# SunYangtian/UniGeo

Measured on AMD Instinct MI355X. Metric: frames/sec (384x512, 25-frame clip, 25 denoise steps), higher is better.
Workload: dtype fp16; 1 GPU; DepthCrafter SVD-UNet fp16, 25-step Euler, 25-frame 384x512 clips (BASELINE configs[1]); CLIP + VAE enc/dec + depth post-proc inside the timed region; one clip per ug_dc_run call, one call at a time (SURVEY 8d; reference eval.py:33-39); frames=25, height=384, width=512, denoise_steps=25, parallelism=clip-sharded x1, RCCL all_gather of depth, clips_in_flight_per_gpu=1, lanes=1

## Files before the change

unigeo_amd/_lib.py:

```python
import ctypes as C
import dataclasses
import json
import os

import numpy as np

_HERE = os.path.dirname(os.path.abspath(__file__))
LIB_PATH = os.environ.get("UG_LIB_PATH") or os.path.join(_HERE, "csrc", "libunigeo_hip.so")

EXPORTS = [
    "ug_unet_config_default", "ug_vae_config_default", "ug_clip_config_default",
    "ug_create", "ug_destroy", "ug_last_error", "ug_workspace_peak",
    "ug_load_tensor", "ug_bind_unet", "ug_bind_vae", "ug_bind_clip",
    "ug_dc_set_inputs", "ug_dc_run", "ug_dc_run_windows", "ug_dc_get_outputs", "ug_dc_device_ptrs", "ug_dc_set_trace", "ug_dc_set_guidance", "ug_unet_forward_pair", "ug_dc_set_inputs_ex", "ug_dc_get_noise", "ug_op_philox_u32", "ug_op_randn", "ug_op_u8_to_frames", "ug_set_vae_encode_fp32", "ug_set_concurrency", "ug_set_coscheduled", "ug_set_fp8_linears", "ug_op_linear_mx8", "ug_set_ff_fused", "ug_op_ff", "ug_op_ln_ff", "ug_bench_ff", "ug_bench_flash", "ug_tune_flash", "ug_tune_ff",
    "ug_eval_depth", "ug_eval_normal", "ug_depth_eval_opts_default", "ug_eval_depth_ex", "ug_eval_depth_global", "ug_op_masked_median", "ug_clip_embed", "ug_vae_encode", "ug_vae_decode", "ug_unet_forward", "ug_normals_from_depth",
    "ug_op_linear", "ug_op_conv", "ug_op_conv_gn", "ug_op_groupnorm", "ug_op_layernorm", "ug_op_flash_attn",
    "ug_op_temporal_attn", "ug_op_attention_generic", "ug_op_flash_attn_dh", "ug_op_euler_step", "ug_op_flash_cross_attn", "ug_op_temporal_attn_nv",
    "ug_op_split_pair", "ug_op_gn32_pair", "ug_op_conv_wide", "ug_op_attn_wide",
    "ug_bind_stablenormal", "ug_sn_run", "ug_sn_unet_forward", "ug_sn_dino", "ug_sn_vae_decode", "ug_sn_vae_encode", "ug_resize_bilinear",
    "ug_pcd_opts_default", "ug_pcd_world_points", "ug_eval_pcd", "ug_op_pcd_nn", "ug_op_pcd_select", "ug_op_pcd_knn_normals", "ug_eval_pcd_fps", "ug_op_pcd_fps",
    "ug_eval_pcd_ex", "ug_op_pcd_nn_grid", "ug_op_pcd_knn_normals_grid",
    "ug_pointmap_opts_default", "ug_pointmap_focal", "ug_pointmap_poses",
    "ug_vis_depth_range", "ug_vis_panels", "ug_prep_resize_frames", "ug_prep_gt", "ug_prep_gt_ex",
    "ug_profile_begin", "ug_profile_begin_shapes", "ug_profile_end", "ug_bench_gemm", "ug_bench_groupnorm", "ug_bench_mfma_peak", "ug_tune_force",
]


class UNetConfigC(C.Structure):
    _fields_ = [("in_channels", C.c_int), ("out_channels", C.c_int), ("num_levels", C.c_int),
                ("block_out_channels", C.c_int * 8), ("num_attention_heads", C.c_int * 8),
                ("down_has_attn", C.c_int * 8),
                ("layers_per_block", C.c_int), ("cross_attention_dim", C.c_int),
                ("addition_time_embed_dim", C.c_int), ("projection_class_embeddings_input_dim", C.c_int),
                ("norm_groups", C.c_int),
                ("eps_cross_attn_blocks", C.c_float), ("eps_plain_down_block", C.c_float),
                ("eps_mid_block", C.c_float), ("eps_up_blocks", C.c_float)]


class VAEConfigC(C.Structure):
    _fields_ = [("in_channels", C.c_int), ("out_channels", C.c_int), ("latent_channels", C.c_int),
                ("num_levels", C.c_int), ("block_out_channels", C.c_int * 8),
                ("layers_per_block", C.c_int), ("norm_groups", C.c_int), ("scaling_factor", C.c_float)]


class CLIPConfigC(C.Structure):
    _fields_ = [("hidden_size", C.c_int), ("intermediate_size", C.c_int), ("num_hidden_layers", C.c_int),
                ("num_attention_heads", C.c_int), ("image_size", C.c_int), ("patch_size", C.c_int),
                ("projection_dim", C.c_int), ("layer_norm_eps", C.c_float)]


class DepthEvalOptsC(C.Structure):
    _fields_ = [("alignment", C.c_int), ("max_depth", C.c_float), ("pre_clip_min", C.c_float), ("pre_clip_max", C.c_float),
                ("post_clip_min", C.c_float), ("post_clip_max", C.c_float)]


class PcdOptsC(C.Structure):
    _fields_ = [("threshold", C.c_float), ("max_iteration", C.c_int), ("knn", C.c_int)]


class PointmapOptsC(C.Structure):
    _fields_ = [("reproj_px", C.c_double), ("max_iter", C.c_int), ("max_rounds", C.c_int)]


DEPTH_ALIGNMENTS = {"lstsq": 0, "median": 1, "scale": 2, "metric": 3}
PREP_DEPTH_F64, PREP_ZOOMED = 1, 2

_lib = None


def _set_argtypes(lib, table):
    try:
        for name, argtypes in table.items():
            getattr(lib, name).argtypes = argtypes
    except AttributeError:
        if not os.environ.get("UG_LIB_PATH"):
            raise


def load_library():
    global _lib
    if _lib is not None:
        return _lib
    if not os.path.exists(LIB_PATH):
        raise RuntimeError(
            f"{LIB_PATH} not found: build it with `python -c 'import __graft_entry__ as g; g.build()'` "
            "(or `make -C unigeo_amd/csrc`).  The MI355X path has no CPU / PyTorch fallback.")
    lib = C.CDLL(LIB_PATH)
    fp, ip, vp = C.POINTER(C.c_float), C.c_int, C.c_void_p
    lib.ug_create.restype = vp
    lib.ug_create.argtypes = [ip, C.c_size_t, C.c_size_t]
    lib.ug_destroy.argtypes = [vp]
    lib.ug_last_error.restype = C.c_char_p
    lib.ug_last_error.argtypes = [vp]
    lib.ug_workspace_peak.restype = C.c_size_t
    lib.ug_workspace_peak.argtypes = [vp]
    lib.ug_load_tensor.argtypes = [vp, C.c_char_p, ip, ip, C.POINTER(C.c_int64), vp]
    lib.ug_bind_unet.argtypes = [vp, C.POINTER(UNetConfigC)]
    lib.ug_bind_vae.argtypes = [vp, C.POINTER(VAEConfigC)]
    lib.ug_bind_clip.argtypes = [vp, C.POINTER(CLIPConfigC)]
    lib.ug_dc_set_inputs.argtypes = [vp, vp, ip, ip, ip, vp, vp, vp]
    lib.ug_dc_run.argtypes = [vp, ip, ip, ip]
    lib.ug_dc_run_windows.argtypes = [vp, ip, ip, ip, ip, ip]
    lib.ug_dc_get_outputs.argtypes = [vp, vp, vp, vp]
    lib.ug_dc_set_trace.argtypes = [vp, vp, ip]
    lib.ug_set_vae_encode_fp32.argtypes = [vp, ip]
    _set_argtypes(lib, {
        "ug_set_fp8_linears": [vp, ip], "ug_set_concurrency": [vp, ip], "ug_set_coscheduled": [vp, ip], "ug_set_ff_fused": [vp, ip],
        "ug_bench_ff": [vp, ip, ip, ip, ip, vp], "ug_bench_flash": [vp, ip, ip, ip, ip, ip, vp], "ug_tune_flash": [vp, ip], "ug_tune_ff": [vp, ip],
        "ug_op_ff": [vp, vp, ip, ip, vp, vp, vp, vp, vp, C.c_float, C.c_float, ip, vp],
        "ug_op_ln_ff": [vp, vp, ip, ip, vp, vp, C.c_float, vp, ip, vp, vp, vp, vp, C.c_float, C.c_float, ip, vp],
        "ug_op_linear_mx8": [vp, vp, ip, ip, vp, ip, vp, ip, vp, vp, vp]})
    _set_argtypes(lib, {"ug_dc_set_guidance": [vp, C.c_float], "ug_unet_forward_pair": [vp, vp, vp, vp, vp, ip, ip, ip, C.c_float, vp, vp]})
    _set_argtypes(lib, {
        "ug_dc_set_inputs_ex": [vp, vp, ip, ip, ip, ip, vp, vp, C.c_uint64, vp], "ug_dc_get_noise": [vp, vp, vp],
        "ug_op_philox_u32": [vp, C.c_uint64, C.c_uint32, C.c_uint64, C.c_long, vp],
        "ug_op_randn": [vp, C.c_uint64, C.c_uint32, C.c_uint64, C.c_long, C.c_long, vp], "ug_op_u8_to_frames": [vp, vp, ip, ip, ip, vp]})
    lib.ug_dc_device_ptrs.argtypes = [vp, C.POINTER(vp), C.POINTER(vp), C.POINTER(vp)]
    lib.ug_eval_depth.argtypes = [vp, vp, vp, vp, C.c_long, C.c_float, vp]
    lib.ug_eval_normal.argtypes = [vp, vp, vp, vp, C.c_long, vp]
    lib.ug_depth_eval_opts_default.restype = None
    lib.ug_depth_eval_opts_default.argtypes = [C.POINTER(DepthEvalOptsC)]
    lib.ug_eval_depth_ex.argtypes = [vp, vp, vp, vp, C.c_long, C.POINTER(DepthEvalOptsC), vp, vp]
    lib.ug_eval_depth_global.argtypes = [vp, vp, vp, vp, vp, vp, vp, ip, ip, ip, C.POINTER(DepthEvalOptsC), vp, vp]
    lib.ug_op_masked_median.argtypes = [vp, vp, vp, C.c_long, C.c_float, C.c_float, C.c_float, vp, C.POINTER(C.c_long)]
    lib.ug_pcd_opts_default.restype = None
    _set_argtypes(lib, {"ug_pcd_opts_default": [C.POINTER(PcdOptsC)],
                        "ug_pcd_world_points": [vp, vp, vp, vp, vp, ip, ip, ip, C.POINTER(DepthEvalOptsC), vp, vp],
                        "ug_eval_pcd": [vp, vp, vp, vp, C.c_long, vp, C.c_long, C.POINTER(PcdOptsC), vp, vp, vp],
                        "ug_op_pcd_nn": [vp, vp, C.c_long, vp, C.c_long, vp, vp, vp],
                        "ug_op_pcd_select": [vp, vp, ip, C.c_long, C.c_long, vp],
                        "ug_op_pcd_knn_normals": [vp, vp, C.c_long, ip, vp, vp]})
    _set_argtypes(lib, {"ug_eval_pcd_fps": [vp, vp, vp, vp, C.c_long, C.c_long, C.POINTER(PcdOptsC), vp, vp, vp, vp, vp],
                        "ug_op_pcd_fps": [vp, vp, C.c_long, C.c_long, vp, vp]})
    _set_argtypes(lib, {"ug_eval_pcd_ex": [vp, vp, vp, vp, C.c_long, vp, C.c_long, C.POINTER(PcdOptsC), ip, vp, vp, vp, vp, vp, vp],
                        "ug_op_pcd_nn_grid": [vp, vp, C.c_long, vp, C.c_long, vp, vp, vp, vp],
                        "ug_op_pcd_knn_normals_grid": [vp, vp, C.c_long, ip, vp, vp, vp]})
    _set_argtypes(lib, {"ug_pointmap_opts_default": [C.POINTER(PointmapOptsC)],
                        "ug_pointmap_focal": [vp, vp, ip, ip, C.c_double, C.c_double, vp],
                        "ug_pointmap_poses": [vp, vp, vp, ip, ip, ip, C.c_double, C.c_double, C.c_double, C.POINTER(PointmapOptsC), vp, vp, vp, vp]})
    if hasattr(lib, "ug_pointmap_opts_default"):
        lib.ug_pointmap_opts_default.restype = None
    _set_argtypes(lib, {"ug_vis_depth_range": [vp, vp, C.c_long, vp],
                        "ug_vis_panels": [vp, vp, vp, vp, ip, ip, ip, ip, C.c_float, C.c_float, vp, vp, ip, vp]})
    _set_argtypes(lib, {"ug_prep_resize_frames": [vp, vp, ip, ip, ip, ip, ip, vp, vp, ip, vp, vp, ip, vp],
                        "ug_prep_gt": [vp, vp, C.c_float, vp, vp, vp, ip, ip, ip, vp, ip, vp, ip, C.c_float, vp, vp, vp, vp, vp],
                        "ug_prep_gt_ex": [vp, vp, C.c_float, vp, vp, vp, ip, ip, ip, vp, ip, vp, ip, C.c_float, vp, vp, vp, vp, vp, C.c_uint]})
    lib.ug_clip_embed.argtypes = [vp, vp, ip, ip, ip, vp]
    lib.ug_vae_encode.argtypes = [vp, vp, ip, ip, ip, vp]
    lib.ug_vae_decode.argtypes = [vp, vp, ip, ip, ip, vp]
    lib.ug_unet_forward.argtypes = [vp, vp, ip, ip, ip, C.c_float, vp, vp]
    lib.ug_normals_from_depth.argtypes = [vp, vp, vp, ip, ip, ip, vp]
    lib.ug_op_linear.argtypes = [vp, vp, ip, ip, vp, ip, vp, vp, C.c_float, C.c_float, ip, ip, vp]
    lib.ug_op_conv.argtypes = [vp, vp, ip, vp, ip, ip, ip, ip, vp, vp, ip, ip, ip, ip, ip, ip, ip, vp]
    lib.ug_op_groupnorm.argtypes = [vp, vp, ip, vp, ip, ip, ip, ip, C.c_float, ip, ip, vp, vp, vp]
    lib.ug_op_conv_gn.argtypes = [vp, vp, ip, ip, ip, ip, vp, vp, vp, ip, ip, ip, ip, C.c_float, ip, vp, vp, vp, vp, vp, vp]
    lib.ug_op_layernorm.argtypes = [vp, vp, ip, ip, C.c_float, vp, vp, vp, ip, vp, vp]
    lib.ug_op_flash_attn.argtypes = [vp, vp, ip, ip, ip, vp]
    lib.ug_op_temporal_attn.argtypes = [vp, vp, ip, ip, ip, vp]
    lib.ug_op_attention_generic.argtypes = [vp, vp, ip, ip, ip, ip, vp]
    lib.ug_op_flash_attn_dh.argtypes = [vp, vp, ip, ip, ip, ip, vp]
    lib.ug_op_euler_step.argtypes = [vp, vp, vp, C.c_long, C.c_float, C.c_float]
    _set_argtypes(lib, {"ug_op_flash_cross_attn": [vp, vp, vp, ip, ip, ip, ip, ip, C.c_long, C.c_long, C.c_long, C.c_long, vp],
                        "ug_op_temporal_attn_nv": [vp, vp, ip, ip, ip, ip, vp]})
    _set_argtypes(lib, {
        "ug_op_split_pair": [vp, vp, C.c_long, ip, vp, vp], "ug_op_gn32_pair": [vp, vp, ip, ip, ip, ip, C.c_float, ip, vp, vp, vp, vp],
        "ug_op_conv_wide": [vp, vp, ip, ip, ip, ip, vp, vp, ip, vp, ip, ip, ip, ip, ip, vp], "ug_op_attn_wide": [vp, vp, ip, ip, ip, vp]})
    lib.ug_bind_stablenormal.argtypes = [vp, C.POINTER(UNetConfigC), C.POINTER(VAEConfigC), C.POINTER(CLIPConfigC)]
    lib.ug_sn_run.argtypes = [vp, vp, ip, ip, ip, vp, C.c_float, ip, vp, vp, vp, vp]
    lib.ug_sn_unet_forward.argtypes = [vp, ip, vp, vp, ip, ip, ip, C.c_float, C.c_float, vp, vp, ip, vp]
    lib.ug_sn_dino.argtypes = [vp, vp, ip, ip, ip, vp]
    lib.ug_sn_vae_decode.argtypes = [vp, vp, ip, ip, ip, vp]
    lib.ug_sn_vae_encode.argtypes = [vp, vp, ip, ip, ip, vp]
    lib.ug_resize_bilinear.argtypes = [vp, vp, ip, ip, ip, ip, ip, ip, ip, vp]
    lib.ug_profile_begin.argtypes = [vp]
    lib.ug_bench_gemm.argtypes = [vp] + [ip] * 16 + [vp]
    lib.ug_bench_groupnorm.argtypes = [vp, ip, ip, ip, ip, ip, ip, ip, vp]
    lib.ug_bench_mfma_peak.argtypes = [vp, ip, vp]
    lib.ug_tune_force.argtypes = [vp, ip, ip]
    lib.ug_profile_begin_shapes.argtypes = [vp]
    lib.ug_profile_end.restype = C.c_char_p
    lib.ug_profile_end.argtypes = [vp]
    _lib = lib
    return lib


def _f32(a):
    return np.ascontiguousarray(a, dtype=np.float32)


def _ptr(a):
    return None if a is None else a.ctypes.data_as(C.c_void_p)


def _fill8(dst, vals):
    for i in range(8):
        dst[i] = int(vals[i]) if i < len(vals) else 0


def _unet_c(cfg):
    c = UNetConfigC()
    c.in_channels, c.out_channels, c.num_levels = cfg.in_channels, cfg.out_channels, len(cfg.block_out_channels)
    _fill8(c.block_out_channels, cfg.block_out_channels)
    _fill8(c.num_attention_heads, cfg.num_attention_heads)
    _fill8(c.down_has_attn, [int(b) for b in cfg.down_has_attn])
    c.layers_per_block, c.cross_attention_dim, c.norm_groups = cfg.layers_per_block, cfg.cross_attention_dim, cfg.norm_groups
    for name in ("addition_time_embed_dim", "projection_class_embeddings_input_dim",
                 "eps_cross_attn_blocks", "eps_plain_down_block", "eps_mid_block", "eps_up_blocks"):
        setattr(c, name, getattr(cfg, name, 0))
    return c


def _vae_c(cfg):
    c = VAEConfigC()
    c.in_channels, c.out_channels, c.latent_channels = cfg.in_channels, cfg.out_channels, cfg.latent_channels
    c.num_levels = len(cfg.block_out_channels)
    _fill8(c.block_out_channels, cfg.block_out_channels)
    c.layers_per_block, c.norm_groups, c.scaling_factor = cfg.layers_per_block, cfg.norm_groups, cfg.scaling_factor
    return c


def _clip_c(cfg):
    c = CLIPConfigC()
    c.hidden_size, c.intermediate_size = cfg.hidden_size, cfg.intermediate_size
    c.num_hidden_layers, c.num_attention_heads = cfg.num_hidden_layers, cfg.num_attention_heads
    c.image_size, c.patch_size, c.layer_norm_eps = cfg.image_size, cfg.patch_size, cfg.layer_norm_eps
    c.projection_dim = getattr(cfg, "projection_dim", 0)
    return c


class Engine:

    def __init__(self, device_id=0, workspace_bytes=2 << 30, persist_bytes=1 << 30):
        self.lib = load_library()
        self.ctx = self.lib.ug_create(int(device_id), int(workspace_bytes), int(persist_bytes))
        if not self.ctx:
            raise RuntimeError("ug_create failed: " + self.lib.ug_last_error(None).decode())
        self.device_id = device_id

    def close(self):
        if getattr(self, "ctx", None):
            self.lib.ug_destroy(self.ctx)
            self.ctx = None

    def __del__(self):
        try:
            self.close()
        except Exception:
            pass

    def _ck(self, rc):
        if rc != 0:
            raise RuntimeError("libunigeo_hip: " + self.lib.ug_last_error(self.ctx).decode())

    def load_state(self, prefix, state):
        for name, arr in state.items():
            a = np.ascontiguousarray(arr)
            if a.dtype == np.float16:
                dt = 0
            elif a.dtype == np.float32:
                dt = 1
            else:
                a = a.astype(np.float32); dt = 1
            shape = (C.c_int64 * max(a.ndim, 1))(*(a.shape if a.ndim else (1,)))
            self._ck(self.lib.ug_load_tensor(self.ctx, (prefix + name).encode(), dt, max(a.ndim, 1), shape, _ptr(a)))

    def bind_unet(self, cfg):
        self._ck(self.lib.ug_bind_unet(self.ctx, C.byref(_unet_c(cfg))))
        self.unet_cfg = cfg

    def bind_vae(self, cfg):
        self._ck(self.lib.ug_bind_vae(self.ctx, C.byref(_vae_c(cfg))))
        self.vae_cfg = cfg

    def bind_clip(self, cfg):
        self._ck(self.lib.ug_bind_clip(self.ctx, C.byref(_clip_c(cfg))))
        self.clip_cfg = cfg

    def bind_stablenormal(self, ucfg, vcfg, dcfg):
        self._ck(self.lib.ug_bind_stablenormal(self.ctx, C.byref(_unet_c(ucfg)), C.byref(_vae_c(vcfg)), C.byref(_clip_c(dcfg))))
        self.sn_cfgs = (ucfg, vcfg, dcfg)

    def sn_run(self, images, prompt_embeds, yoso_t, timesteps, ca, cb):
        f = _f32(images); B, H, W, _ = f.shape
        pe = _f32(prompt_embeds).reshape(77, self.sn_cfgs[0].cross_attention_dim)
        ts, a, b = _f32(timesteps), _f32(ca), _f32(cb)
        out = np.empty((B, H, W, 3), np.float32)
        self._ck(self.lib.ug_sn_run(self.ctx, _ptr(f), B, H, W, _ptr(pe), float(yoso_t), int(ts.size), _ptr(ts), _ptr(a), _ptr(b), _ptr(out)))
        return out

    def sn_unet_forward(self, which, sample, t_unet, prompt_embeds, zimg=None, t_ctrl=0.0, dino_tokens=None, use_ctrl=False):
        s = _f32(sample); B, _, h, w = s.shape
        z = None if zimg is None else _f32(zimg)
        d = None if dino_tokens is None else _f32(dino_tokens)
        pe = _f32(prompt_embeds)
        out = np.empty((B, 4, h, w), np.float32)
        self._ck(self.lib.ug_sn_unet_forward(self.ctx, int(which), _ptr(s), _ptr(z), B, h, w, float(t_unet), float(t_ctrl), _ptr(pe), _ptr(d),
                                             int(bool(use_ctrl)), _ptr(out)))
        return out

    def sn_dino(self, images):
        f = _f32(images); B, H, W, _ = f.shape
        dc = self.sn_cfgs[2]; g = dc.image_size // dc.patch_size
        out = np.empty((B, g * g, dc.hidden_size), np.float32)
        self._ck(self.lib.ug_sn_dino(self.ctx, _ptr(f), B, H, W, _ptr(out)))
        return out

    def sn_vae_decode(self, z):
        z = _f32(z); B, _, h, w = z.shape
# ... 402 lines not shown
        return out[0]

    def op_pcd_knn_normals(self, pts, knn=30):
        p = np.ascontiguousarray(np.asarray(pts, np.float64).reshape(-1, 3))
        nbr, nrm = np.empty((len(p), min(knn, len(p))), np.int32), np.empty((len(p), 3), np.float64)
        self._ck(self.lib.ug_op_pcd_knn_normals(self.ctx, _ptr(p), len(p), int(knn), _ptr(nbr), _ptr(nrm)))
        return nbr, nrm

    def op_masked_median(self, pred, gt, max_depth=80.0, pre_clip_min=None, pre_clip_max=None):
        p, g = _f32(pred).reshape(-1), _f32(gt).reshape(-1)
        med = np.zeros(2, np.float32); cnt = C.c_long(0)
        nan = float("nan")
        self._ck(self.lib.ug_op_masked_median(self.ctx, _ptr(p), _ptr(g), p.size, nan if max_depth is None else float(max_depth),
                                              nan if pre_clip_min is None else float(pre_clip_min),
                                              nan if pre_clip_max is None else float(pre_clip_max), _ptr(med), C.byref(cnt)))
        return med[0], med[1], int(cnt.value)

    def eval_normal(self, gt, mask=None, pred=None):
        g = _f32(gt); n = g.size // 3
        p = None if pred is None else _f32(pred)
        m = None if mask is None else np.ascontiguousarray(np.asarray(mask).astype(np.uint8))
        out = np.zeros(8, np.float64)
        self._ck(self.lib.ug_eval_normal(self.ctx, _ptr(p), _ptr(g), _ptr(m), n, _ptr(out)))
        return dict(zip(self.NORMAL_KEYS, out.tolist()))

    VIS_RGB_NONE, VIS_RGB_HOST, VIS_RGB_RESIDENT = 0, 1, 2

    def vis_depth_range(self, depth=None):
        out = np.zeros(2, np.float32)
        if depth is None:
            T, H, W = self._shape
            self._ck(self.lib.ug_vis_depth_range(self.ctx, None, T * H * W, _ptr(out)))
        else:
            d = _f32(depth)
            self._ck(self.lib.ug_vis_depth_range(self.ctx, _ptr(d), d.size, _ptr(out)))
        return out[0], out[1]

    def vis_panels(self, vmin, vmax, lut, depth=None, normals=None, rgbs=None, cbar=None):
        d = None if depth is None else _f32(depth)
        n = None if normals is None else _f32(normals)
        if d is not None:
            shape = d.shape
        elif n is not None:
            shape = n.shape[:3]
        else:
            shape = self._shape
        if len(shape) != 3 or (n is not None and n.shape != (*shape, 3)):
            raise ValueError("vis_panels: depth must be [T,H,W] and normals [T,H,W,3]")
        T, H, W = shape
        r, mode = None, self.VIS_RGB_NONE
        if isinstance(rgbs, str):
            if rgbs != "resident":
                raise ValueError('vis_panels: rgbs must be None, "resident" or an array')
            mode = self.VIS_RGB_RESIDENT
        elif rgbs is not None:
            r, mode = _f32(rgbs), self.VIS_RGB_HOST
            if r.shape != (T, H, W, 3):
                raise ValueError("vis_panels: rgbs must be [T,H,W,3]")
        l = _f32(lut)
        if l.shape != (256, 3):
            raise ValueError("vis_panels: lut must be [256,3]")
        cb, Wc = None, 0
        if cbar is not None:
            cb = _f32(cbar)
            if cb.ndim != 3 or cb.shape[0] != H or cb.shape[2] != 3:
                raise ValueError("vis_panels: cbar must be [H,Wc,3]")
            Wc = cb.shape[1]
        Wp = (W if mode else 0) + 2 * W + (5 + Wc if cb is not None else 0)
        out = np.empty((T, H, Wp, 3), np.uint8)
        self._ck(self.lib.ug_vis_panels(self.ctx, _ptr(d), _ptr(n), _ptr(r), mode, T, H, W, float(vmin), float(vmax), _ptr(l), _ptr(cb), Wc, _ptr(out)))
        return out

    def prep_resize_frames(self, frames_u8, Ho, Wo, row_taps=None, col_taps=None):
        from .harness.scannetpp import resize_taps
        f = np.asarray(frames_u8)
        if f.dtype != np.uint8 or f.ndim != 4 or f.shape[3] != 3:
            raise ValueError("prep_resize_frames: frames must be uint8 [T,Hi,Wi,3]")
        f = np.ascontiguousarray(f)
        T, Hi, Wi, _ = f.shape
        Ho, Wo = int(Ho), int(Wo)
        tabs = []
        for taps, n_in, n_out in ((row_taps, Hi, Ho), (col_taps, Wi, Wo)):
            idx, w = resize_taps(n_in, n_out) if taps is None else taps
            idx, w = np.ascontiguousarray(idx, dtype=np.int32), np.ascontiguousarray(w, dtype=np.float64)
            if idx.ndim != 2 or idx.shape != w.shape or idx.shape[0] != n_out:
                raise ValueError("prep_resize_frames: a tap table must be (idx, w), both [n_out, K]")
            tabs.append((idx, w))
        (ri, rw), (ci, cw) = tabs
        out = np.empty((T, 3, Ho, Wo), np.float32)
        self._ck(self.lib.ug_prep_resize_frames(self.ctx, _ptr(f), T, Hi, Wi, Ho, Wo, _ptr(ri), _ptr(rw), ri.shape[1], _ptr(ci), _ptr(cw),
                                                ci.shape[1], _ptr(out)))
        return out

    def prep_gt(self, depth_u16, normals_u8, intrinsics, cam2key, row_idx, col_idx, depth_divisor=1000.0, max_depth=80.0, depth_f64=False,
                zoomed=None):
        d = np.asarray(depth_u16)
        if d.dtype != np.uint16 or d.ndim != 3:
            raise ValueError("prep_gt: depth must be uint16 [T,Hi,Wi]")
        d = np.ascontiguousarray(d)
        T, Hi, Wi = d.shape
        n = None
        if normals_u8 is not None:
            n = np.asarray(normals_u8)
            if n.dtype != np.uint8 or n.shape != (T, Hi, Wi, 3):
                raise ValueError("prep_gt: normals must be uint8 [T,Hi,Wi,3]")
            n = np.ascontiguousarray(n)
        k, m = _f32(intrinsics).reshape(T, 3, 3), _f32(cam2key).reshape(T, 4, 4)
        ri, ci = np.ascontiguousarray(row_idx, dtype=np.int32).reshape(-1), np.ascontiguousarray(col_idx, dtype=np.int32).reshape(-1)
        Ho, Wo = ri.size, ci.size
        cn, cc, wn, wc = (np.empty((T, 3, Ho, Wo), np.float32) for _ in range(4))
        mask = np.empty((T, Ho, Wo), np.float32)
        if zoomed is None:
            zoomed = (Ho, Wo) != (Hi, Wi)
        flags = (PREP_DEPTH_F64 if depth_f64 else 0) | (PREP_ZOOMED if zoomed else 0)
        self._ck(self.lib.ug_prep_gt_ex(self.ctx, _ptr(d), float(depth_divisor), _ptr(n), _ptr(k), _ptr(m), T, Hi, Wi, _ptr(ri), Ho, _ptr(ci), Wo,
                                        float(max_depth), _ptr(cn), _ptr(cc), _ptr(wn), _ptr(wc), _ptr(mask), flags))
        return cn, cc, wn, wc, mask

    def op_linear(self, A, W, bias=None, R1=None, c0=1.0, c1=1.0, act=0, geglu=False):
        A, W = _f32(A), _f32(W); M, K = A.shape; N = W.shape[0]
        b = None if bias is None else _f32(bias); r = None if R1 is None else _f32(R1)
        out = np.empty((M, N // 2 if geglu else N), np.float32)
        self._ck(self.lib.ug_op_linear(self.ctx, _ptr(A), M, K, _ptr(W), N, _ptr(b), _ptr(r), c0, c1, act, int(geglu), _ptr(out)))
        return out

    def op_conv(self, x0, weight, bias=None, x1=None, kt=1, k=3, stride=1, pad_t=1, pad_l=1, ups=1):
        x0 = _f32(x0); T, H, W, C0 = x0.shape
        x1a = None if x1 is None else _f32(x1); C1 = 0 if x1 is None else x1a.shape[-1]
        w = _f32(weight); O = w.shape[0]
        b = None if bias is None else _f32(bias)
        Ho, Wo = H * ups // stride, W * ups // stride
        out = np.empty((T, Ho, Wo, O), np.float32)
        self._ck(self.lib.ug_op_conv(self.ctx, _ptr(x0), C0, _ptr(x1a), C1, T, H, W, _ptr(w), _ptr(b), O, kt, k,
                                     stride, pad_t, pad_l, ups, _ptr(out)))
        return out

    def op_groupnorm(self, x0, G, eps, gamma, beta, x1=None, temporal=False, silu=False):
        x0 = _f32(x0); T, HW, C0 = x0.shape
        x1a = None if x1 is None else _f32(x1); C1 = 0 if x1 is None else x1a.shape[-1]
        out = np.empty((T, HW, C0 + C1), np.float32)
        self._ck(self.lib.ug_op_groupnorm(self.ctx, _ptr(x0), C0, _ptr(x1a), C1, T, HW, G, eps, int(temporal), int(silu),
                                          _ptr(_f32(gamma)), _ptr(_f32(beta)), _ptr(out)))
        return out

    def op_conv_gn(self, x, w, b, G, eps, gamma, beta, res=None, kt=1, k=3, temporal=False):
        x = _f32(x); T, H, W, C0 = x.shape; w = _f32(w); O = w.shape[0]
        r = None if res is None else _f32(res)
        co = np.empty((T, H, W, O), np.float32); y1 = np.empty_like(co); y2 = np.empty_like(co)
        rb = C.c_int(0)
        self._ck(self.lib.ug_op_conv_gn(self.ctx, _ptr(x), C0, T, H, W, _ptr(w), _ptr(None if b is None else _f32(b)), _ptr(r), O, kt, k, G, eps, int(temporal),
                                        _ptr(_f32(gamma)), _ptr(_f32(beta)), _ptr(co), _ptr(y1), _ptr(y2), C.byref(rb)))
        return co, y1, y2, rb.value

    def op_layernorm(self, x, eps, gamma, beta, addvec=None, rows_per_vec=1):
        x = _f32(x); M, Cc = x.shape
        out = np.empty((M, Cc), np.float32); xout = np.empty((M, Cc), np.float32)
        av = None if addvec is None else _f32(addvec)
        self._ck(self.lib.ug_op_layernorm(self.ctx, _ptr(x), M, Cc, eps, _ptr(_f32(gamma)), _ptr(_f32(beta)), _ptr(av),
                                          rows_per_vec, _ptr(out), _ptr(xout)))
        return (out, xout) if addvec is not None else out

    def op_flash_attn(self, qkv, B, H, S):
        q = _f32(qkv); out = np.empty((B * S, H * 64), np.float32)
        self._ck(self.lib.ug_op_flash_attn(self.ctx, _ptr(q), B, H, S, _ptr(out)))
        return out

    def op_temporal_attn(self, qkv, T, HW, H):
        q = _f32(qkv); out = np.empty((T * HW, H * 64), np.float32)
        self._ck(self.lib.ug_op_temporal_attn(self.ctx, _ptr(q), T, HW, H, _ptr(out)))
        return out

    def op_flash_cross_attn(self, q, kv, out_inout, B, H, S, Sk=0, kv_shared=False, guard=0):
        q, kv, out = _f32(q), _f32(kv), np.array(out_inout, dtype=np.float32, order="C")
        keys = Sk if Sk > 0 else S
        assert q.ndim == kv.ndim == out.ndim == 2 and q.shape[0] == B * S and out.shape[0] == B * S + guard, (q.shape, kv.shape, out.shape)
        assert Sk < 0 or kv.shape[0] == (1 if kv_shared else B) * keys + guard, kv.shape
        self._ck(self.lib.ug_op_flash_cross_attn(self.ctx, _ptr(q), _ptr(kv), B, H, S, Sk, int(bool(kv_shared)), q.shape[1], kv.shape[1], out.shape[1],
                                                 int(guard), _ptr(out)))
        return out

    def op_temporal_attn_nv(self, qkv, nv, T, HW, H):
        q = _f32(qkv); out = np.empty((nv * T * HW, H * 64), np.float32)
        assert q.shape == (nv * T * HW, 3 * H * 64), q.shape
        self._ck(self.lib.ug_op_temporal_attn_nv(self.ctx, _ptr(q), nv, T, HW, H, _ptr(out)))
        return out

    def op_attention_generic(self, qkv, B, S, H, d):
        q = _f32(qkv); out = np.empty((B * S, H * d), np.float32)
        self._ck(self.lib.ug_op_attention_generic(self.ctx, _ptr(q), B, S, H, d, _ptr(out)))
        return out

    def op_flash_attn_dh(self, qkv, B, S, H, d):
        q = _f32(qkv); out = np.empty((B * S, H * d), np.float32)
        self._ck(self.lib.ug_op_flash_attn_dh(self.ctx, _ptr(q), B, S, H, d, _ptr(out)))
        return out

    def op_split_pair(self, x):
        x = _f32(x); M, Cc = x.shape
        hi = np.empty((M, Cc), np.float32); lo = np.empty((M, Cc), np.float32)
        self._ck(self.lib.ug_op_split_pair(self.ctx, _ptr(x), M, Cc, _ptr(hi), _ptr(lo)))
        return hi, lo

    def op_gn32_pair(self, x, G, eps, gamma, beta, silu=False):
        x = _f32(x); T, HW, Cc = x.shape
        hi = np.empty((T, HW, Cc), np.float32); lo = np.empty((T, HW, Cc), np.float32)
        self._ck(self.lib.ug_op_gn32_pair(self.ctx, _ptr(x), T, HW, Cc, G, eps, int(silu), _ptr(_f32(gamma)), _ptr(_f32(beta)), _ptr(hi), _ptr(lo)))
        return hi, lo

    def op_conv_wide(self, x, weight, bias=None, res=None, res_in_place=False, k=3, stride=1, pad_t=1, pad_l=1):
        x = _f32(x); T, H, W, Cc = x.shape
        w = _f32(weight); O = w.shape[0]
        b = None if bias is None else _f32(bias); r = None if res is None else _f32(res)
        out = np.empty((T, H // stride, W // stride, O), np.float32)
        self._ck(self.lib.ug_op_conv_wide(self.ctx, _ptr(x), T, H, W, Cc, _ptr(w), _ptr(b), O, _ptr(r), int(bool(res_in_place)), k, stride, pad_t, pad_l, _ptr(out)))
        return out

    def op_attn_wide(self, qkv, T, S):
        q = _f32(qkv); Cc = q.shape[1] // 3
        out = np.empty((T * S, Cc), np.float32)
        self._ck(self.lib.ug_op_attn_wide(self.ctx, _ptr(q), T, S, Cc, _ptr(out)))
        return out

    def op_euler_step(self, v, lat, sigma, sigma_next):
        v = _f32(v); l = _f32(lat).copy()
        self._ck(self.lib.ug_op_euler_step(self.ctx, _ptr(v), _ptr(l), l.size, sigma, sigma_next))
        return l

    def bench_gemm(self, M=0, N=0, K=0, conv=None, cfg=-1, split=0, iters=20):
        out = np.zeros(8, np.float32)
        cv = conv or {}
        self._ck(self.lib.ug_bench_gemm(self.ctx, M, N, K, int(conv is not None), cv.get("T", 0), cv.get("H", 0), cv.get("W", 0),
                                        cv.get("C0", 0), cv.get("C1", 0), cv.get("kt", 1), cv.get("k", 1), cv.get("stride", 1),
                                        cv.get("ups", 1), cfg, split, iters, _ptr(out)))
        Mr, Kr = float(out[3]), float(out[4])
        return float(out[0]), 2.0 * Mr * N * Kr / (out[0] * 1e-3) / 1e12, int(out[1]), int(out[2])

    def bench_mfma_peak(self, iters=20000):
        out = np.zeros(1, np.float32)
        self._ck(self.lib.ug_bench_mfma_peak(self.ctx, int(iters), _ptr(out)))
        return float(out[0])

    def tune_force(self, cfg=-1, split=-1):
        self._ck(self.lib.ug_tune_force(self.ctx, int(cfg), int(split)))

    def bench_groupnorm(self, C0, C1, T, HW, temporal, mode, iters=20):
        out = np.zeros(1, np.float32)
        self._ck(self.lib.ug_bench_groupnorm(self.ctx, C0, C1, T, HW, int(temporal), mode, iters, _ptr(out)))
        return float(out[0])

    def profile_begin(self, shapes=False):
        self._ck((self.lib.ug_profile_begin_shapes if shapes else self.lib.ug_profile_begin)(self.ctx))

    def profile_end(self):
        prof = json.loads(self.lib.ug_profile_end(self.ctx).decode())
        self.last_profile_order = prof.pop("__order__", None)
        return prof

    def workspace_peak(self):
        return int(self.lib.ug_workspace_peak(self.ctx))
```

unigeo_amd/csrc/common.h:

```cpp
#pragma once
#include <hip/hip_runtime.h>
#include <hip/hip_fp16.h>
#include <stdint.h>
#include <stdio.h>
#include <stdexcept>
#include <string>

typedef _Float16 f16;
typedef _Float16 f16x2 __attribute__((ext_vector_type(2)));
typedef _Float16 f16x4 __attribute__((ext_vector_type(4)));
typedef _Float16 f16x8 __attribute__((ext_vector_type(8)));
typedef float f32x4 __attribute__((ext_vector_type(4)));
typedef float f32x16 __attribute__((ext_vector_type(16)));

#define UG_CHECK(expr)                                                                        \
  do {                                                                                        \
    hipError_t _e = (expr);                                                                   \
    if (_e != hipSuccess)                                                                     \
      throw std::runtime_error(std::string(#expr) + " failed: " + hipGetErrorString(_e) +    \
                               " at " + __FILE__ + ":" + std::to_string(__LINE__));           \
  } while (0)

#define UG_REQUIRE(cond, msg)                                                                 \
  do {                                                                                        \
    if (!(cond))                                                                              \
      throw std::runtime_error(std::string("requirement failed: ") + #cond + " : " + (msg) + \
                               " at " + __FILE__ + ":" + std::to_string(__LINE__));           \
  } while (0)

static inline int cdiv(long a, long b) { return (int)((a + b - 1) / b); }
static inline int ug_dev_slot() { int d = 0; (void)hipGetDevice(&d); return d & 31; }

enum { UG_ACT_NONE = 0, UG_ACT_SILU = 1, UG_ACT_GELU = 2 };
enum { UG_F_GEGLU = 1, UG_F_OUT_F32 = 2, UG_F_NOXCD = 4, UG_F_PRIO = 8 ,
       UG_F_XCDROUND = 32 ,
       UG_F_R1_F32 = 16  };

struct GemmP {
  const f16* A0; const f16* A1;
  int C0, C1;
  int M, N, K;
  int conv;
  int T, Hi, Wi, Ho, Wo;
  int ups, stride, pad_t, pad_l;
  int kt, ky, kx;
  const f16* W; long ldw;
  const f16* bias; const f16* bias2;
  const f16* R1; long ldr1; float c1;
  const f16* R2; long ldr2; float c2;
  float c0;
  void* Out; long ldo;
  int act, flags;
  const f16* zero;
  int nb_inner;
  long sA_o, sA_i, sW_o, sW_i, sO_o, sO_i;
  int cfg_p1;
  int splitk;
  float* partial;
  void* trace;
  int up_phase;
  const unsigned* sa; const unsigned* sw; long ld_sa, ld_sw;
  int kchunk;
  int tm_T, tm_nb;
  int m_off;
  int group_m;
  int halo_tw, halo_lg;
  int tune_cfg_p1, tune_split_p1, tune_knobs;
  float2* stat_part; int stat_hw;
};
struct GemmTune { int cfg = -1, split = -1, knobs = 0; };
static inline void gemm_apply_tune(GemmP& p, const GemmTune& t) { p.tune_cfg_p1 = t.cfg + 1; p.tune_split_p1 = t.split + 1; p.tune_knobs = t.knobs; }
void launch_gemm_mx8(const GemmP& p, hipStream_t s);
void launch_quant_mx8(const f16* x, long ldx, long M, int K, unsigned char* q, unsigned* scales, long ld_s, hipStream_t s);
void launch_gemm(const GemmP& p, int batch, hipStream_t s, int* stat_rb = nullptr);
bool gemm_stream_supported(const GemmP& p, int batch);
void launch_gemm_stream(const GemmP& p, hipStream_t s);
bool conv_halo_supported(const GemmP& p, int batch, int bm, int bn);
void launch_conv_halo(const GemmP& p, int bm, int bn, hipStream_t s);
void gemm_plan(const GemmP& p, int batch, int* cfg_out, int* split_out);

struct FFusedP {
  const f16* X; const f16* W1; const f16* b1; const f16* W2; const f16* b2;
  const f16* R1; const f16* R2; float c0, c1, c2;
  f16* Out; int M, C; const f16* zero;
  const f16* ln_g; const f16* ln_b; float ln_eps; const f16* addvec; int rows_per_vec;
  int variant;
};
bool ff_fused_supported(int C);
void launch_ff_fused(const FFusedP& p, hipStream_t s);

struct GroupNormP {
  const f16* X0; const f16* X1; int C0, C1;
  int T, HW, G; float eps; int temporal; int silu;
  const f16* gamma; const f16* beta;
  f16* Y;
  float* ws;
  int mode;
  const float2* part; int part_rb;
};
bool launch_groupnorm(const GroupNormP& p, hipStream_t s);
bool groupnorm_uses_part(const GroupNormP& p, int part_rb);
size_t groupnorm_ws_floats(int T, int HW, int C, int G);

struct LayerNormP {
  const f16* X; f16* Y; int M, C; float eps;
  const f16* gamma; const f16* beta;
  const f16* addvec; int rows_per_vec; f16* Xout;
  long row0;
  unsigned char* Y8; unsigned* S8; long ld_s8;
};
void launch_layernorm(const LayerNormP& p, hipStream_t s);

struct FlashP {
  const f16* Q; const f16* K; const f16* V; long ldq, ldk, ldv;
  f16* O; long ldo;
  int B, H, S; float scale;
  int Sk = 0; int kv_shared = 0;
  int variant = -1;
};
void launch_flash_attn64(const FlashP& p, hipStream_t s);
bool flash_attn_dh_supported(int d);
void launch_flash_attn_dh(const FlashP& p, int d, hipStream_t s);

struct TemporalAttnP {
  const f16* Q; const f16* K; const f16* V; long ld;
  f16* O; long ldo;
  int T, HW, H; float scale;
  int nv = 1;
};
void launch_temporal_attn64(const TemporalAttnP& p, hipStream_t s);

void launch_softmax_rows(const float* in, long ld_in, f16* out, long ld_out, long rows, int S,
                         hipStream_t s);
void launch_transpose(const f16* in, long ldi, long sbi, f16* out, long ldo, long sbo, int B, int R,
                      int C, int nb_inner, long sbi_inner, long sbo_inner, hipStream_t s);

void launch_cast_f32_f16(const float* in, f16* out, long n, hipStream_t s);
void launch_cast_f16_f32(const f16* in, float* out, long n, hipStream_t s);
void launch_permute_conv_w(const f16* in, f16* out, int O, int I, int taps, int Ipad, int Opad,
                           hipStream_t s);
void launch_upsample_phase_w(const f16* w9, f16* w4, int O, int I, int Ipad, hipStream_t s);
void launch_rechunk_conv_w(const f16* in, f16* out, long O, int taps, int Ipad, hipStream_t s);
void launch_gather_rows(const f16* in, f16* out, const int* rowmap, int rows, int cols, hipStream_t s);
void launch_copy2d(const f16* in, long ldi, f16* out, long ldo, long rows, int cols, hipStream_t s);
void launch_fill_f16(f16* p, float v, long n, hipStream_t s);
void launch_fill_random(f16* p, long n, unsigned seed, hipStream_t s);
void launch_add_rowvec(const f16* x, const f16* vec, f16* y, long M, int C, int rows_per_vec,
                       hipStream_t s);
void launch_axpby(const f16* a, const f16* b, f16* y, float ca, float cb, long n, hipStream_t s);

void launch_prep_video(const float* frames, const float* noise, f16* clip_src, f16* vae_in,
                       int T, int H, int W, float noise_aug, hipStream_t s);
void launch_clip_patchify(const f16* video_m11, f16* patches, int T, int H, int W, int S224,
                          int P, int Kpad, hipStream_t s, int imagenet_norm = 0);
void launch_scale_rows(f16* w, const f16* gamma, int N, int K, hipStream_t s);
void launch_add_grid_nearest(f16* x, const f16* grid, int B, int h, int w, int g, int C, hipStream_t s);
void launch_sn_normals_out(const f16* dec, int ldd, float* out, long pixels, hipStream_t s);
void launch_resize_bilinear_aa(const float* in, float* out, int B, int Hi, int Wi, int Ho, int Wo, int C, int normalise, hipStream_t s);
void launch_init_latents2(const float* noise, f16* lat, float sigma0, int T, long hw, hipStream_t s);
void launch_silu_f16(const f16* in, f16* out, long n, hipStream_t s);
void launch_clip_assemble(const f16* patches, const f16* cls, const f16* pos, f16* tok, int T, int np, int d,
                          hipStream_t s);
void launch_make_unet_input(const f16* lat, const f16* cond, f16* x, long pixels, float inv_scale,
                            hipStream_t s);
void launch_euler_step(const f16* v, f16* lat, long n, float sigma, float sigma_next, hipStream_t s);
void launch_make_unet_input_cfg(const f16* lat, const f16* cond, f16* x, long pixels, float inv_scale, hipStream_t s);
void launch_euler_step_cfg(const f16* vc, const f16* vu, float g, f16* lat, long n, float sigma, float sigma_next, hipStream_t s);
void launch_scale_f16(const f16* in, f16* out, float sc, long n, hipStream_t s);
void launch_axpby_f16(const f16* x, float a, const f16* y, float b, f16* out, long n, hipStream_t s);
void launch_crossfade_f16(const f16* cur, f16* all, long frame_elems, int overlap, hipStream_t s);
void launch_pad_channels(const f16* in, int Cin, f16* out, int Cout, long pixels, hipStream_t s);
void launch_time_conv_out(const f16* x, const f16* w, const f16* b, float* frames_out, int T,
                          long HW, int Cs, hipStream_t s);
void launch_depth_post(const float* frames, float* depth, float* minmax_ws, long pixels,
                       hipStream_t s);
void launch_normals(const float* depth, const float* K33, float* normals, int T, int H, int W,
                    hipStream_t s);

void launch_philox_u32(uint32_t* out, long nblocks, uint64_t seed, uint32_t stream, uint64_t q0, hipStream_t s);
void launch_randn(float* out, long n, uint64_t seed, uint32_t stream, uint64_t e0, hipStream_t s);
void launch_u8_to_frames(const unsigned char* in_tchw, float* out_thwc, int T, long HW, hipStream_t s);

void launch_split_pair(const float* x, f16* y, long M, int C, hipStream_t s);
void launch_add_f32(const float* a, const float* b, float* y, long n, hipStream_t s);
void launch_take_cols_f16(const float* x, long ldx, f16* y, long M, int C, hipStream_t s);
size_t gn32_ws_bytes(int T, int HW, int C, int G);
void launch_gn32_pair(const float* X, f16* Y, int T, int HW, int C, int G, float eps, int silu, const f16* gamma, const f16* beta,
                      void* ws, hipStream_t s);
void launch_qk_terms(const float* qkv, f16* Aq, f16* Bk, long M, int C, hipStream_t s);
void launch_vt_terms(const float* qkv, f16* Vt, int B, int S, int Spad, int C, hipStream_t s);
void launch_softmax_pair(const float* in, long ld_in, f16* out, int Spad, long rows, int S, float pscale, hipStream_t s);

float bench_mfma_peak(float* scratch, int iters, hipStream_t s);

void launch_depth_fit(const float* pred, const float* gt, long n, float max_depth, double* part, int* nb, hipStream_t s);
void launch_depth_metrics(const float* pred, const float* gt, const unsigned char* cmask, long n, float max_depth, float sc,
                          float sh, double* part, int* nb, hipStream_t s);
void launch_normal_err(const float* pn, const float* gn, const unsigned char* mask, long n, float* err, double* part,
                       unsigned* hist, int* nb, hipStream_t s);
void launch_collect_bin(const float* err, long n, int bin, float* out, unsigned* count, unsigned cap, hipStream_t s);
#define SEL_PREFIX 2048
#define SEL_RANK 2050
#define SEL_COUNT 2052
#define SEL_MED 2053
#define SEL_WORDS 2056
void launch_masked_median(const float* pred, const float* gt, long n, float max_depth, float lo, float hi, unsigned* sel, hipStream_t s);
void launch_weiszfeld_scale(const float* pred, const float* gt, long n, float max_depth, float lo, float hi, int iters, double* wz,
                            double* part, hipStream_t s);
void launch_depth_fit_ex(const float* pred, const float* gt, long n, float max_depth, float lo, float hi, double* part, int* nb, hipStream_t s);
void launch_depth_metrics_ex(const float* pred, const float* gt, const unsigned char* cmask, long n, float max_depth, float lo, float hi,
                             float plo, float phi, float sc, float sh, double* part, float* emap, int* nb, hipStream_t s);
void launch_world_radius(const float* pred, const float* gt, const float* gt_radius, const double* cam, long n, int H, int W, float max_depth,
                         float plo, float phi, float sc, float sh, float* radius, double* part, int* nb, hipStream_t s);
void launch_world_points(const float* pred, const double* cam, long n, int H, int W, float plo, float phi, float sc, float sh, float* pts,
                         hipStream_t s);
void launch_radius_metrics(const float* radius, const float* gt, const float* gt_radius, const unsigned char* cmask, long n, float max_depth,
                           float sc, float sh, double* part, float* rmap, int* nb, hipStream_t s);
#define PCD_MAXB 1024
#define PCD_SEL_WORDS 264
__host__ __device__ inline unsigned long long pcd_key(double f) {
  const unsigned long long u = __builtin_bit_cast(unsigned long long, f);
  return u ^ ((u >> 63) ? ~0ull : (1ull << 63));
}
__host__ __device__ inline unsigned long long pcd_key(float f) {
  const unsigned u = __builtin_bit_cast(unsigned, f);
  return (unsigned long long)(u ^ ((u >> 31) ? 0xffffffffu : 0x80000000u)) << 32;
}
__host__ __device__ inline double pcd_unkey_f64(unsigned long long k) {
  return __builtin_bit_cast(double, k ^ ((k >> 63) ? (1ull << 63) : ~0ull));
}
__host__ __device__ inline float pcd_unkey_f32(unsigned long long k) {
// ... 65 lines not shown
```

unigeo_amd/csrc/engine.h:

```cpp
#pragma once
#include <map>
#include <memory>
#include <string>
#include <unordered_map>
#include <vector>

#include "common.h"

namespace ug {

struct RawTensor { void* dev = nullptr; int dtype = 0; std::vector<long> shape; long numel = 0; bool used = false; };

class Arena {
 public:
  void init(size_t bytes);
  void destroy();
  void* alloc(size_t bytes);
  template <class T> T* get(long n) { return (T*)alloc((size_t)n * sizeof(T)); }
  size_t mark() const { return off_; }
  void release(size_t m) { off_ = m; }
  size_t peak() const { return peak_; }
  size_t capacity() const { return cap_; }
  void view(void* base, size_t bytes) { base_ = (char*)base; cap_ = bytes; off_ = 0; peak_ = 0; hi_ = 0; }
  void reset_high() { hi_ = off_; }
  size_t high() const { return hi_; }
  void note_peak(size_t p) { if (p > peak_) peak_ = p; }
 private:
  char* base_ = nullptr; size_t cap_ = 0, off_ = 0, peak_ = 0, hi_ = 0;
};

struct Lin { const f16* w = nullptr; const f16* b = nullptr; int in = 0, out = 0;
             const unsigned char* w8 = nullptr; const unsigned* sw8 = nullptr; long ld_sw8 = 0; };
struct Conv { const f16* w = nullptr; const f16* b = nullptr; int cin = 0, cinp = 0, cout = 0, kt = 1, ky = 1, kx = 1;
              const f16* wphase = nullptr;
              int kchunk = 0; };
struct Norm { const f16* g = nullptr; const f16* b = nullptr; int c = 0; float eps = 1e-5f; };

struct Res2D { Norm n1, n2; Conv c1, c2, sc; Lin temb; bool has_sc = false, has_temb = false; int tidx = -1; };
struct ResT { Norm n1, n2; Conv c1, c2; Lin temb; bool has_temb = false; int tidx = -1; };
struct STRes { Res2D s; ResT t; float alpha = 0.5f; int cin = 0, cout = 0; };

struct Transformer {
  int C = 0, heads = 0;
  Norm gn; Lin proj_in, proj_out;
  Norm ln1, ln3; Lin qkv1, o1, v2, o2, ff1, ff2;
  Norm ln_in, tln1, tln3; Lin ffin1, ffin2, tqkv, to1, tv2, to2, tff1, tff2;
  Lin tpe1, tpe2;
  float alpha = 0.5f;
  f16* frame_emb = nullptr; int frame_emb_T = 0;
  f16* cross_sp = nullptr;
  f16* cross_tm = nullptr;
};

struct UNetCfg {
  int in_ch = 8, out_ch = 4, nlev = 4; int boc[8] = {320, 640, 1280, 1280}; int heads[8] = {5, 10, 20, 20};
  int has_attn[8] = {1, 1, 1, 0}; int layers = 2, cross_dim = 1024, add_dim = 256, proj_in_dim = 768, groups = 32;
  float eps_xattn = 1e-6f, eps_down = 1e-5f, eps_mid = 1e-5f, eps_up = 1e-6f;
};
struct VAECfg { int in_ch = 3, out_ch = 3, lat = 4, nlev = 4; int boc[8] = {128, 256, 512, 512}; int layers = 2, groups = 32; float scaling = 0.18215f; };
struct CLIPCfg { int hidden = 1280, inter = 5120, layers = 32, heads = 16, image = 224, patch = 14, proj = 1024; float eps = 1e-5f; };

struct UNet {
  UNetCfg cfg; bool bound = false;
  Conv conv_in, conv_out; Norm norm_out;
  Lin te1, te2, ae1, ae2;
  struct Down { std::vector<STRes> res; std::vector<Transformer> attn; Conv down; bool has_down = false; };
  struct Up { std::vector<STRes> res; std::vector<Transformer> attn; Conv up; bool has_up = false; };
  std::vector<Down> down; std::vector<Up> up;
  STRes mid0, mid1; Transformer mid_attn;
  std::vector<Res2D*> temb_s; std::vector<ResT*> temb_t;
  f16* tproj = nullptr; long tproj_stride = 0; int tproj_steps = 0; std::vector<long> tproj_off_s, tproj_off_t;
  int prep_nv = 1;
};

struct VAttn { Norm gn; Lin qkv, out; int C = 0; };
struct VAE {
  VAECfg cfg; bool bound = false;
  Conv e_in, e_out, quant; Norm e_norm;
  struct EDown { std::vector<Res2D> res; Conv down; bool has_down = false; };
  std::vector<EDown> edown; Res2D emid0, emid1; VAttn eattn;
  std::vector<EDown> edown_w; Res2D emid0_w, emid1_w; VAttn eattn_w; Conv e_out_w, quant_w; bool wide_bound = false;
  Conv d_in, d_out; Norm d_norm; const f16* tco_w = nullptr; const f16* tco_b = nullptr;
  std::vector<STRes> dmid; VAttn dattn;
  struct DUp { std::vector<STRes> res; Conv up; bool has_up = false; };
  std::vector<DUp> dup;
  bool dec2d = false; Conv post_quant; std::vector<Res2D> d2_mid; std::vector<std::vector<Res2D>> d2_up;
};

struct CLIPLayer { Norm ln1, ln2; Lin qkv, out, fc1, fc2; };
struct CLIP {
  CLIPCfg cfg; bool bound = false;
  const f16* patch_w = nullptr; int patch_k = 0;
  const f16* patch_b = nullptr;
  const f16* cls = nullptr; const f16* pos = nullptr;
  Norm pre, post; std::vector<CLIPLayer> layers; Lin proj;
};

struct SDTransformer {
  int C = 0, heads = 0;
  Norm gn; Lin proj_in, proj_out; Norm ln1, ln2, ln3; Lin qkv1, o1, q2, kv2, o2, ff1, ff2;
  f16* kv = nullptr;
};
struct TembSet { std::vector<Res2D*> res; f16* tproj = nullptr; std::vector<long> off; int steps = 0; };
struct SDTrunk {
  Conv conv_in; Lin te1, te2;
  struct Down { std::vector<Res2D> res; std::vector<SDTransformer> attn; Conv down; bool has_down = false; };
  std::vector<Down> down; Res2D mid0, mid1; SDTransformer mid_attn;
};
struct SDUNetM {
  SDTrunk tr; TembSet ts;
  struct Up { std::vector<Res2D> res; std::vector<SDTransformer> attn; Conv up; bool has_up = false; };
  std::vector<Up> up; Norm norm_out; Conv conv_out;
};
struct ControlNetM { SDTrunk tr; TembSet ts; std::vector<Conv> zero; Conv zero_mid; Lin dino_proj; bool has_dino = false; };
struct SN {
  UNetCfg cfg; bool bound = false;
  SDUNetM unet_y, unet_r; ControlNetM ctrl_y, ctrl_d; VAE vae; CLIP dino;
};

struct ProfRec { std::string name; double flops, bytes; hipEvent_t e0, e1; };

struct Lane { hipStream_t stream = nullptr; hipEvent_t done = nullptr; };

struct Ctx {
  int device = 0; hipStream_t stream = nullptr;
  Arena ws;
  Arena persist;
  f16* zero = nullptr;
  std::string err;
  std::unordered_map<std::string, RawTensor> raw;
  UNet unet; VAE vae; CLIP clip; SN sn;
  bool prof_on = false; bool prof_shapes = false; std::vector<ProfRec> prof; std::string prof_json;
  int T = 0, H = 0, W = 0;
  float* d_frames = nullptr; float* d_noise_lat = nullptr; float* d_noise_aug = nullptr; float* d_K = nullptr;
  float* d_out_frames = nullptr; float* d_depth = nullptr; float* d_normals = nullptr; float* d_mm = nullptr;
  f16* d_clip_emb = nullptr; f16* d_cond = nullptr; f16* d_lat = nullptr;
  size_t io_mark = 0; bool io_ready = false;
  bool normals_ready = false;
  float* d_pcd_pts = nullptr; long pcd_cap = 0, pcd_pixels = 0;
  float* trace_host = nullptr; int trace_steps = 0;
  void* pin[2] = {nullptr, nullptr}; size_t pin_sz[2] = {0, 0};
  int ff_fused = 3;
  int fp8_linears = 0;
  int vae_encode_fp32 = 1;
  float guidance = 1.f;
  std::vector<Lane> lanes; hipEvent_t fork_ev = nullptr;
  int concurrency = 1;
  std::map<std::string, size_t> lane_need;
  int cur_lane = 0;
  int cosched = 0;
  int ff_variant = 0, flash_variant = -1;
  GemmTune tune;
};

void* pinned(Ctx& c, int slot, size_t bytes);

void upload_raw(Ctx& c, const std::string& name, int dtype, const std::vector<long>& shape, const void* host);
void bind_unet(Ctx& c, const UNetCfg& cfg, const std::string& prefix);
void bind_vae(Ctx& c, const VAECfg& cfg, const std::string& prefix);
void bind_clip(Ctx& c, const CLIPCfg& cfg, const std::string& prefix);
void finish_binding(Ctx& c, const std::string& prefix);
inline int geglu_src_row(int v, int inner) { const int blk = v / 16, wv = v % 16; return wv < 8 ? blk * 8 + wv : inner + blk * 8 + (wv - 8); }

void unet_prepare(Ctx& c, int T, const f16* clip_emb, const float* timesteps, int nsteps, int nv = 1);
f16* unet_forward(Ctx& c, const f16* x, int T, int h, int w, int step, int nv = 1, int vid0 = 0);
f16* vae_encode(Ctx& c, const f16* x8, int T, int H, int W);
void vae_decode(Ctx& c, const f16* z, int T, int h, int w, float* frames_out);
f16* clip_embed(Ctx& c, const f16* video_m11, int T, int H, int W);

f16* vae_encode_v(Ctx& c, VAE& v, const f16* x8, int T, int H, int W, bool fp32_grade);
void test_unfused_attention(Ctx& c, const f16* qkv, long ld, int B, int S, int H, int d, f16* out, long ldo);
void attn_wide_core(Ctx& c, const float* qkv, int T, int S, int C, float* ao);
void test_conv_wide(Ctx& c, const std::string& name, bool bias, const float* x, int T, int H, int W, int cin, int cout, int k, int stride, int pad_t, int pad_l,
                    float* out, const float* res);

void bind_sn(Ctx& c, const UNetCfg& ucfg, const VAECfg& vcfg, const CLIPCfg& dcfg, const std::string& prefix);
void sn_run(Ctx& c, const float* images, int B, int H, int W, const float* prompt, float yoso_t, int nsteps, const float* timesteps,
            const float* ca, const float* cb, float* normals_out);
f16* sn_unet_eval(Ctx& c, int which, const f16* sample4, const f16* zimg4, int B, int h, int w, float t_unet, float t_ctrl, const f16* prompt,
                  const f16* dino_tok, int use_ctrl);
f16* sn_dino_tokens(Ctx& c, const f16* img_m11, int B, int H, int W);
f16* sn_vae_decode(Ctx& c, const f16* z4, int B, int h, int w);

void dc_set_inputs(Ctx& c, const float* frames, int T, int H, int W, const float* noise_lat, const float* noise_aug,
                   const float* K33);
void dc_set_inputs_ex(Ctx& c, const void* frames, int frames_u8, int T, int H, int W, const float* noise_lat, const float* noise_aug,
                      uint64_t noise_seed, const float* K33);
void dc_get_noise(Ctx& c, float* noise_lat, float* noise_aug);
// ... 8 lines not shown
```

unigeo_amd/csrc/engine.hip:

```cpp
#include "engine.h"
#include <chrono>

#include <math.h>
#include <stdlib.h>
#include <string.h>

#include <algorithm>
#include <exception>
#include <sstream>

namespace ug {

void Arena::init(size_t bytes) {
  UG_CHECK(hipMalloc((void**)&base_, bytes));
  cap_ = bytes; off_ = 0; peak_ = 0;
}
void Arena::destroy() { if (base_) (void)hipFree(base_); base_ = nullptr; cap_ = 0; }
void* Arena::alloc(size_t bytes) {
  const size_t a = (bytes + 255) & ~(size_t)255;
  if (off_ + a > cap_)
    throw std::runtime_error("device arena exhausted: need " + std::to_string(off_ + a) + " bytes, capacity " +
                             std::to_string(cap_) + " (raise workspace_bytes / persist_bytes in ug_create)");
  void* p = base_ + off_;
  off_ += a;
// ... 348 lines not shown
  f16* d = c.persist.get<f16>(t.numel);
  if (t.dtype == 0) UG_CHECK(hipMemcpyAsync(d, t.dev, (size_t)t.numel * 2, hipMemcpyDeviceToDevice, c.stream));
  else launch_cast_f32_f16((const float*)t.dev, d, t.numel, c.stream);
  return d;
}
static const f16* persist_f16(Ctx& c, RawTensor& t) { return raw_f16(c, t, true); }

static float raw_scalar(Ctx& c, const std::string& name) {
  RawTensor& t = raw_get(c, name, {1});
  UG_CHECK(hipStreamSynchronize(c.stream));
  if (t.dtype == 1) { float v; UG_CHECK(hipMemcpy(&v, t.dev, 4, hipMemcpyDeviceToHost)); return v; }
  uint16_t h; UG_CHECK(hipMemcpy(&h, t.dev, 2, hipMemcpyDeviceToHost));
  f16 hv; memcpy(&hv, &h, 2);
  return (float)hv;
}

static Norm bind_norm(Ctx& c, const std::string& p, int ch, float eps) {
  Norm n; n.c = ch; n.eps = eps;
  n.g = persist_f16(c, raw_get(c, p + ".weight", {ch}));
  n.b = persist_f16(c, raw_get(c, p + ".bias", {ch}));
  return n;
}
static Lin bind_lin(Ctx& c, const std::string& p, int in, int out, bool bias) {
  Lin l; l.in = in; l.out = out;
  l.w = persist_f16(c, raw_get(c, p + ".weight", {out, in}));
  l.b = bias ? persist_f16(c, raw_get(c, p + ".bias", {out})) : nullptr;
  return l;
}
static Lin bind_lin_cat(Ctx& c, const std::vector<std::string>& ps, int in, int out_each, bool bias) {
  Lin l; l.in = in; l.out = out_each * (int)ps.size();
  f16* w = c.persist.get<f16>((long)l.out * in);
  f16* b = bias ? c.persist.get<f16>(l.out) : nullptr;
  for (size_t i = 0; i < ps.size(); ++i) {
    RawTensor& t = raw_get(c, ps[i] + ".weight", {out_each, in});
    const size_t mk = c.persist.mark();
    const f16* src = raw_f16(c, t, false);
    UG_CHECK(hipMemcpyAsync(w + (long)i * out_each * in, src, (size_t)out_each * in * 2, hipMemcpyDeviceToDevice, c.stream));
    UG_CHECK(hipStreamSynchronize(c.stream));
    c.persist.release(mk);
    if (bias) {
      RawTensor& tb = raw_get(c, ps[i] + ".bias", {out_each});
      const size_t mk2 = c.persist.mark();
      const f16* sb = raw_f16(c, tb, false);
      UG_CHECK(hipMemcpyAsync(b + (long)i * out_each, sb, (size_t)out_each * 2, hipMemcpyDeviceToDevice, c.stream));
      UG_CHECK(hipStreamSynchronize(c.stream));
      c.persist.release(mk2);
    }
  }
  l.w = w; l.b = b;
  return l;
}
static Lin bind_geglu(Ctx& c, const std::string& p, int in, int inner) {
  const int out = 2 * inner;
  UG_REQUIRE(inner % 8 == 0, "GEGLU inner dim must be a multiple of 8");
  RawTensor& tw = raw_get(c, p + ".weight", {out, in});
  RawTensor& tb = raw_get(c, p + ".bias", {out});
  std::vector<int> map(out);
  for (int v = 0; v < out; ++v) map[v] = geglu_src_row(v, inner);
  int* dmap = (int*)c.persist.alloc(out * sizeof(int));
  UG_CHECK(hipMemcpy(dmap, map.data(), out * sizeof(int), hipMemcpyHostToDevice));
  Lin l; l.in = in; l.out = out;
  f16* w = c.persist.get<f16>((long)out * in);
  f16* b = c.persist.get<f16>(out);
  const size_t mk = c.persist.mark();
  launch_gather_rows(raw_f16(c, tw, false), w, dmap, out, in, c.stream);
  launch_gather_rows(raw_f16(c, tb, false), b, dmap, out, 1, c.stream);
  UG_CHECK(hipStreamSynchronize(c.stream));
  c.persist.release(mk);
  l.w = w; l.b = b;
  return l;
}
static inline int pad8(int x) { return (x + 7) & ~7; }
static void quant_lin(Ctx& c, Lin& l) {
  if (l.in % 128 != 0 || l.out < 64) return;
  unsigned char* w8 = (unsigned char*)c.persist.alloc((size_t)l.out * l.in);
  const long ld = pad256(l.out);
  unsigned* sw = (unsigned*)c.persist.alloc((size_t)(l.in / 128) * ld * 4);
  UG_CHECK(hipMemsetAsync(sw, 0, (size_t)(l.in / 128) * ld * 4, c.stream));
  launch_quant_mx8(l.w, l.in, l.out, l.in, w8, sw, ld, c.stream);
  l.w8 = w8; l.sw8 = sw; l.ld_sw8 = ld;
}
static Conv bind_conv(Ctx& c, const std::string& p, int cin, int cout, int kt, int k, bool bias = true, bool upsampler = false) {
  Conv cv; cv.cin = cin; cv.cinp = pad8(cin); cv.cout = cout; cv.kt = kt; cv.ky = k; cv.kx = k;
  RawTensor* t;
  if (kt > 1) t = &raw_get(c, p + ".weight", {cout, cin, kt, 1, 1});
  else t = &raw_get(c, p + ".weight", {cout, cin, k, k});
  const int taps = kt * k * k;
  f16* w = c.persist.get<f16>((long)cout * taps * cv.cinp);
  const size_t mk = c.persist.mark();
  launch_permute_conv_w(raw_f16(c, *t, false), w, cout, cin, taps, cv.cinp, cout, c.stream);
  UG_CHECK(hipStreamSynchronize(c.stream));
  c.persist.release(mk);
  cv.w = w;
  if (upsampler && kt == 1 && k == 3 && !getenv("UG_NO_SUBPIXEL")) {
    f16* w4 = c.persist.get<f16>((long)4 * cout * 4 * cv.cinp);
    const size_t mk2 = c.persist.mark();
    launch_upsample_phase_w(raw_f16(c, *t, false), w4, cout, cin, cv.cinp, c.stream);
    UG_CHECK(hipStreamSynchronize(c.stream));
    c.persist.release(mk2);
    cv.wphase = w4;
  }
  cv.b = bias ? persist_f16(c, raw_get(c, p + ".bias", {cout})) : nullptr;
  if (taps > 1 && cv.cinp % 64 == 0) {
    const size_t mk3 = c.persist.mark();
    f16* tmp = c.persist.get<f16>((long)cout * taps * cv.cinp);
    UG_CHECK(hipMemcpyAsync(tmp, w, (size_t)cout * taps * cv.cinp * 2, hipMemcpyDeviceToDevice, c.stream));
    launch_rechunk_conv_w(tmp, w, cout, taps, cv.cinp, c.stream);
    if (cv.wphase) {
      f16* t4 = c.persist.get<f16>((long)4 * cout * 4 * cv.cinp);
      UG_CHECK(hipMemcpyAsync(t4, cv.wphase, (size_t)4 * cout * 4 * cv.cinp * 2, hipMemcpyDeviceToDevice, c.stream));
      launch_rechunk_conv_w(t4, (f16*)cv.wphase, (long)4 * cout, 4, cv.cinp, c.stream);
    }
    UG_CHECK(hipStreamSynchronize(c.stream));
    c.persist.release(mk3);
    cv.kchunk = 1;
  }
  return cv;
}

static Conv dup_conv(Ctx& c, const Conv& cv) {
  Conv d = cv; d.wphase = nullptr;
  const int taps = cv.kt * cv.ky * cv.kx;
  const long rows = cv.kchunk ? (long)cv.cout : (long)cv.cout * taps;
  const long cols = cv.kchunk ? (long)taps * cv.cinp : cv.cinp;
  f16* w = c.persist.get<f16>(rows * 2 * cols);
  launch_copy2d(cv.w, cols, w, 2 * cols, rows, (int)cols, c.stream);
  launch_copy2d(cv.w, cols, w + cols, 2 * cols, rows, (int)cols, c.stream);
  d.w = w; d.cin = 2 * cv.cinp; d.cinp = 2 * cv.cinp;
  return d;
}
static Lin dup_lin(Ctx& c, const Lin& l) {
  Lin d = l;
  f16* w = c.persist.get<f16>((long)l.out * 2 * l.in);
  launch_copy2d(l.w, l.in, w, 2 * l.in, l.out, l.in, c.stream);
  launch_copy2d(l.w, l.in, w + l.in, 2 * l.in, l.out, l.in, c.stream);
  d.w = w; d.in = 2 * l.in;
  return d;
}
static Res2D dup_res2d(Ctx& c, const Res2D& r) {
  Res2D d = r;
  d.c1 = dup_conv(c, r.c1); d.c2 = dup_conv(c, r.c2);
  if (r.has_sc) d.sc = dup_conv(c, r.sc);
  return d;
}

static Res2D bind_res2d(Ctx& c, const std::string& p, int cin, int cout, int temb, float eps) {
  Res2D r;
  r.n1 = bind_norm(c, p + ".norm1", cin, eps);
  r.c1 = bind_conv(c, p + ".conv1", cin, cout, 1, 3);
  if (temb) { r.temb = bind_lin(c, p + ".time_emb_proj", temb, cout, true); r.has_temb = true; }
  r.n2 = bind_norm(c, p + ".norm2", cout, eps);
  r.c2 = bind_conv(c, p + ".conv2", cout, cout, 1, 3);
  if (cin != cout) { r.sc = bind_conv(c, p + ".conv_shortcut", cin, cout, 1, 1); r.has_sc = true; }
  return r;
}
static ResT bind_rest(Ctx& c, const std::string& p, int ch, int temb, float eps) {
  ResT r;
  r.n1 = bind_norm(c, p + ".norm1", ch, eps);
  r.c1 = bind_conv(c, p + ".conv1", ch, ch, 3, 1);
  if (temb) { r.temb = bind_lin(c, p + ".time_emb_proj", temb, ch, true); r.has_temb = true; }
  r.n2 = bind_norm(c, p + ".norm2", ch, eps);
  r.c2 = bind_conv(c, p + ".conv2", ch, ch, 3, 1);
  return r;
}
static STRes bind_stres(Ctx& c, const std::string& p, int cin, int cout, int temb, float eps, float teps, bool sw) {
  STRes r; r.cin = cin; r.cout = cout;
  r.s = bind_res2d(c, p + ".spatial_res_block", cin, cout, temb, eps);
  r.t = bind_rest(c, p + ".temporal_res_block", cout, temb, teps);
  const float mix = raw_scalar(c, p + ".time_mixer.mix_factor");
  const float a = 1.f / (1.f + expf(-mix));
  r.alpha = sw ? 1.f - a : a;
  return r;
}

static void touch(Ctx& c, const std::string& name, std::initializer_list<long> shape) { raw_get(c, name, shape); }

static Transformer bind_transformer(Ctx& c, const std::string& p, int C, int heads, int cross) {
  Transformer t; t.C = C; t.heads = heads;
  UG_REQUIRE(C / heads == 64 && C % heads == 0, "UNet attention head_dim must be 64");
  t.gn = bind_norm(c, p + ".norm", C, 1e-6f);
  t.proj_in = bind_lin(c, p + ".proj_in", C, C, true);
  t.proj_out = bind_lin(c, p + ".proj_out", C, C, true);
  const std::string b = p + ".transformer_blocks.0", tb = p + ".temporal_transformer_blocks.0";
  t.ln1 = bind_norm(c, b + ".norm1", C, 1e-5f);
  t.qkv1 = bind_lin_cat(c, {b + ".attn1.to_q", b + ".attn1.to_k", b + ".attn1.to_v"}, C, C, false);
  t.o1 = bind_lin(c, b + ".attn1.to_out.0", C, C, true);
  touch(c, b + ".norm2.weight", {C}); touch(c, b + ".norm2.bias", {C});
  touch(c, b + ".attn2.to_q.weight", {C, C}); touch(c, b + ".attn2.to_k.weight", {C, cross});
  t.v2 = bind_lin(c, b + ".attn2.to_v", cross, C, false);
  t.o2 = bind_lin(c, b + ".attn2.to_out.0", C, C, true);
  t.ln3 = bind_norm(c, b + ".norm3", C, 1e-5f);
  t.ff1 = bind_geglu(c, b + ".ff.net.0.proj", C, 4 * C);
  t.ff2 = bind_lin(c, b + ".ff.net.2", 4 * C, C, true);
  t.ln_in = bind_norm(c, tb + ".norm_in", C, 1e-5f);
  t.ffin1 = bind_geglu(c, tb + ".ff_in.net.0.proj", C, 4 * C);
  t.ffin2 = bind_lin(c, tb + ".ff_in.net.2", 4 * C, C, true);
  t.tln1 = bind_norm(c, tb + ".norm1", C, 1e-5f);
  t.tqkv = bind_lin_cat(c, {tb + ".attn1.to_q", tb + ".attn1.to_k", tb + ".attn1.to_v"}, C, C, false);
  t.to1 = bind_lin(c, tb + ".attn1.to_out.0", C, C, true);
  touch(c, tb + ".norm2.weight", {C}); touch(c, tb + ".norm2.bias", {C});
  touch(c, tb + ".attn2.to_q.weight", {C, C}); touch(c, tb + ".attn2.to_k.weight", {C, cross});
  t.tv2 = bind_lin(c, tb + ".attn2.to_v", cross, C, false);
  t.to2 = bind_lin(c, tb + ".attn2.to_out.0", C, C, true);
  t.tln3 = bind_norm(c, tb + ".norm3", C, 1e-5f);
  t.tff1 = bind_geglu(c, tb + ".ff.net.0.proj", C, 4 * C);
  t.tff2 = bind_lin(c, tb + ".ff.net.2", 4 * C, C, true);
  t.tpe1 = bind_lin(c, p + ".time_pos_embed.linear_1", C, 4 * C, true);
  t.tpe2 = bind_lin(c, p + ".time_pos_embed.linear_2", 4 * C, C, true);
  const float mix = raw_scalar(c, p + ".time_mixer.mix_factor");
  t.alpha = 1.f / (1.f + expf(-mix));
  for (Lin* l : {&t.proj_in, &t.proj_out, &t.qkv1, &t.o1, &t.ff1, &t.ff2, &t.ffin1, &t.ffin2, &t.tqkv, &t.to1, &t.tff1, &t.tff2}) quant_lin(c, *l);
  return t;
}

void bind_unet(Ctx& c, const UNetCfg& cfg, const std::string& pre) {
  UNet& u = c.unet; u = UNet(); u.cfg = cfg;
  const int n = cfg.nlev, temb = cfg.boc[0] * 4;
  u.conv_in = bind_conv(c, pre + "conv_in", cfg.in_ch, cfg.boc[0], 1, 3);
  u.te1 = bind_lin(c, pre + "time_embedding.linear_1", cfg.boc[0], temb, true);
  u.te2 = bind_lin(c, pre + "time_embedding.linear_2", temb, temb, true);
  u.ae1 = bind_lin(c, pre + "add_embedding.linear_1", cfg.proj_in_dim, temb, true);
  u.ae2 = bind_lin(c, pre + "add_embedding.linear_2", temb, temb, true);
  u.down.resize(n);
  int ch = cfg.boc[0];
  for (int i = 0; i < n; ++i) {
    const float eps = cfg.has_attn[i] ? cfg.eps_xattn : cfg.eps_down;
    for (int j = 0; j < cfg.layers; ++j) {
      const std::string p = pre + "down_blocks." + std::to_string(i);
      u.down[i].res.push_back(bind_stres(c, p + ".resnets." + std::to_string(j), j == 0 ? ch : cfg.boc[i], cfg.boc[i], temb, eps, eps, false));
      if (cfg.has_attn[i])
        u.down[i].attn.push_back(bind_transformer(c, p + ".attentions." + std::to_string(j), cfg.boc[i], cfg.heads[i], cfg.cross_dim));
    }
    if (i != n - 1) {
      u.down[i].down = bind_conv(c, pre + "down_blocks." + std::to_string(i) + ".downsamplers.0.conv", cfg.boc[i], cfg.boc[i], 1, 3);
      u.down[i].has_down = true;
    }
    ch = cfg.boc[i];
  }
  const int cm = cfg.boc[n - 1];
  u.mid0 = bind_stres(c, pre + "mid_block.resnets.0", cm, cm, temb, cfg.eps_mid, cfg.eps_mid, false);
  u.mid_attn = bind_transformer(c, pre + "mid_block.attentions.0", cm, cfg.heads[n - 1], cfg.cross_dim);
  u.mid1 = bind_stres(c, pre + "mid_block.resnets.1", cm, cm, temb, cfg.eps_mid, cfg.eps_mid, false);
  u.up.resize(n);
  int out = cfg.boc[n - 1];
  const int L = cfg.layers + 1;
  for (int i = 0; i < n; ++i) {
    const int prev = out; out = cfg.boc[n - 1 - i];
    const int cin = cfg.boc[n - 1 - std::min(i + 1, n - 1)];
    const int lev = n - 1 - i;
    for (int j = 0; j < L; ++j) {
      const int skip = (j == L - 1) ? cin : out, rin = (j == 0) ? prev : out;
      const std::string p = pre + "up_blocks." + std::to_string(i);
      u.up[i].res.push_back(bind_stres(c, p + ".resnets." + std::to_string(j), rin + skip, out, temb, cfg.eps_up, cfg.eps_up, false));
      if (cfg.has_attn[lev])
        u.up[i].attn.push_back(bind_transformer(c, p + ".attentions." + std::to_string(j), out, cfg.heads[lev], cfg.cross_dim));
    }
    if (i != n - 1) {
      u.up[i].up = bind_conv(c, pre + "up_blocks." + std::to_string(i) + ".upsamplers.0.conv", out, out, 1, 3, true, true);
      u.up[i].has_up = true;
    }
  }
  u.norm_out = bind_norm(c, pre + "conv_norm_out", cfg.boc[0], 1e-5f);
  u.conv_out = bind_conv(c, pre + "conv_out", cfg.boc[0], cfg.out_ch, 1, 3);
  auto add = [&](STRes& r) {
    if (r.s.has_temb) { r.s.tidx = (int)u.temb_s.size(); u.temb_s.push_back(&r.s); }
    if (r.t.has_temb) { r.t.tidx = (int)u.temb_t.size(); u.temb_t.push_back(&r.t); }
  };
  for (auto& d : u.down) for (auto& r : d.res) add(r);
  add(u.mid0); add(u.mid1);
  for (auto& d : u.up) for (auto& r : d.res) add(r);
  u.bound = true;
}

static VAttn bind_vattn(Ctx& c, const std::string& p, int C) {
  VAttn a; a.C = C;
  a.gn = bind_norm(c, p + ".group_norm", C, 1e-6f);
  a.qkv = bind_lin_cat(c, {p + ".to_q", p + ".to_k", p + ".to_v"}, C, C, true);
  a.out = bind_lin(c, p + ".to_out.0", C, C, true);
  return a;
}

static Res2D bind_res2d(Ctx& c, const std::string& p, int cin, int cout, int temb, float eps);
void bind_vae_into(Ctx& c, VAE& v, const VAECfg& cfg, const std::string& pre, bool temporal_decoder) {
  v = VAE(); v.cfg = cfg;
  const int n = cfg.nlev;
  v.e_in = bind_conv(c, pre + "encoder.conv_in", cfg.in_ch, cfg.boc[0], 1, 3);
  v.edown.resize(n);
  int ch = cfg.boc[0];
  for (int i = 0; i < n; ++i) {
    for (int j = 0; j < cfg.layers; ++j)
      v.edown[i].res.push_back(bind_res2d(c, pre + "encoder.down_blocks." + std::to_string(i) + ".resnets." + std::to_string(j),
                                          j == 0 ? ch : cfg.boc[i], cfg.boc[i], 0, 1e-6f));
    if (i != n - 1) {
      v.edown[i].down = bind_conv(c, pre + "encoder.down_blocks." + std::to_string(i) + ".downsamplers.0.conv", cfg.boc[i], cfg.boc[i], 1, 3);
      v.edown[i].has_down = true;
    }
    ch = cfg.boc[i];
  }
  v.emid0 = bind_res2d(c, pre + "encoder.mid_block.resnets.0", ch, ch, 0, 1e-6f);
  v.eattn = bind_vattn(c, pre + "encoder.mid_block.attentions.0", ch);
  v.emid1 = bind_res2d(c, pre + "encoder.mid_block.resnets.1", ch, ch, 0, 1e-6f);
  v.e_norm = bind_norm(c, pre + "encoder.conv_norm_out", ch, 1e-6f);
  v.e_out = bind_conv(c, pre + "encoder.conv_out", ch, 2 * cfg.lat, 1, 3);
  v.quant = bind_conv(c, pre + "quant_conv", 2 * cfg.lat, 2 * cfg.lat, 1, 1);
  v.d_in = bind_conv(c, pre + "decoder.conv_in", cfg.lat, cfg.boc[n - 1], 1, 3);
  v.dattn = bind_vattn(c, pre + "decoder.mid_block.attentions.0", cfg.boc[n - 1]);
  v.d_norm = bind_norm(c, pre + "decoder.conv_norm_out", cfg.boc[0], 1e-6f);
  v.d_out = bind_conv(c, pre + "decoder.conv_out", cfg.boc[0], cfg.out_ch, 1, 3);
  if (!temporal_decoder) {
    v.post_quant = bind_conv(c, pre + "post_quant_conv", cfg.lat, cfg.lat, 1, 1);
    v.d2_mid.push_back(bind_res2d(c, pre + "decoder.mid_block.resnets.0", cfg.boc[n - 1], cfg.boc[n - 1], 0, 1e-6f));
    v.d2_mid.push_back(bind_res2d(c, pre + "decoder.mid_block.resnets.1", cfg.boc[n - 1], cfg.boc[n - 1], 0, 1e-6f));
    v.dup.resize(n); v.d2_up.resize(n);
    int out2 = cfg.boc[n - 1];
    for (int i = 0; i < n; ++i) {
      const int prev = out2; out2 = cfg.boc[n - 1 - i];
      for (int j = 0; j < cfg.layers + 1; ++j)
        v.d2_up[i].push_back(bind_res2d(c, pre + "decoder.up_blocks." + std::to_string(i) + ".resnets." + std::to_string(j),
                                        j == 0 ? prev : out2, out2, 0, 1e-6f));
      if (i != n - 1) {
        v.dup[i].up = bind_conv(c, pre + "decoder.up_blocks." + std::to_string(i) + ".upsamplers.0.conv", out2, out2, 1, 3, true, true);
        v.dup[i].has_up = true;
      }
    }
    v.dec2d = true;
  }
  if (temporal_decoder) {
  for (int j = 0; j < cfg.layers; ++j)
    v.dmid.push_back(bind_stres(c, pre + "decoder.mid_block.resnets." + std::to_string(j), cfg.boc[n - 1], cfg.boc[n - 1], 0, 1e-6f, 1e-5f, true));
  v.dup.resize(n);
  int out = cfg.boc[n - 1];
  for (int i = 0; i < n; ++i) {
    const int prev = out; out = cfg.boc[n - 1 - i];
    for (int j = 0; j < cfg.layers + 1; ++j)
      v.dup[i].res.push_back(bind_stres(c, pre + "decoder.up_blocks." + std::to_string(i) + ".resnets." + std::to_string(j),
                                        j == 0 ? prev : out, out, 0, 1e-6f, 1e-5f, true));
    if (i != n - 1) {
      v.dup[i].up = bind_conv(c, pre + "decoder.up_blocks." + std::to_string(i) + ".upsamplers.0.conv", out, out, 1, 3, true, true);
      v.dup[i].has_up = true;
    }
  }
  UG_REQUIRE(cfg.out_ch == 3, "time_conv_out kernel is written for 3 output channels");
  v.tco_w = persist_f16(c, raw_get(c, pre + "decoder.time_conv_out.weight", {3, 3, 3, 1, 1}));
  v.tco_b = persist_f16(c, raw_get(c, pre + "decoder.time_conv_out.bias", {3}));
  }
  v.edown_w.resize(n);
  for (int i = 0; i < n; ++i) {
    for (auto& r : v.edown[i].res) v.edown_w[i].res.push_back(dup_res2d(c, r));
    v.edown_w[i].has_down = v.edown[i].has_down;
    if (v.edown[i].has_down) v.edown_w[i].down = dup_conv(c, v.edown[i].down);
  }
  v.emid0_w = dup_res2d(c, v.emid0); v.emid1_w = dup_res2d(c, v.emid1);
  v.eattn_w = v.eattn; v.eattn_w.qkv = dup_lin(c, v.eattn.qkv); v.eattn_w.out = dup_lin(c, v.eattn.out);
  v.e_out_w = dup_conv(c, v.e_out); v.quant_w = dup_conv(c, v.quant);
  UG_CHECK(hipStreamSynchronize(c.stream));
  v.wide_bound = true;
  v.bound = true;
}
void bind_vae(Ctx& c, const VAECfg& cfg, const std::string& pre) { bind_vae_into(c, c.vae, cfg, pre, true); }

void bind_clip(Ctx& c, const CLIPCfg& cfg, const std::string& pre) {
  CLIP& m = c.clip; m = CLIP(); m.cfg = cfg;
  const int d = cfg.hidden, P = cfg.patch, ntok = (cfg.image / P) * (cfg.image / P) + 1;
  UG_REQUIRE((d / cfg.heads) % 8 == 0, "CLIP head_dim must be a multiple of 8");
  const std::string v = pre + "vision_model.";
  m.cls = persist_f16(c, raw_get(c, v + "embeddings.class_embedding", {d}));
  m.pos = persist_f16(c, raw_get(c, v + "embeddings.position_embedding.weight", {ntok, d}));
  {
    RawTensor& t = raw_get(c, v + "embeddings.patch_embedding.weight", {d, 3, P, P});
    const int K = 3 * P * P; m.patch_k = pad8(K);
    f16* w = c.persist.get<f16>((long)d * m.patch_k);
    const size_t mk = c.persist.mark();
    launch_permute_conv_w(raw_f16(c, t, false), w, d, K, 1, m.patch_k, d, c.stream);
    UG_CHECK(hipStreamSynchronize(c.stream));
    c.persist.release(mk);
    m.patch_w = w;
  }
  m.pre = bind_norm(c, v + "pre_layrnorm", d, cfg.eps);
  for (int i = 0; i < cfg.layers; ++i) {
    const std::string p = v + "encoder.layers." + std::to_string(i);
    CLIPLayer l;
    l.ln1 = bind_norm(c, p + ".layer_norm1", d, cfg.eps);
    l.qkv = bind_lin_cat(c, {p + ".self_attn.q_proj", p + ".self_attn.k_proj", p + ".self_attn.v_proj"}, d, d, true);
    l.out = bind_lin(c, p + ".self_attn.out_proj", d, d, true);
    l.ln2 = bind_norm(c, p + ".layer_norm2", d, cfg.eps);
    l.fc1 = bind_lin(c, p + ".mlp.fc1", d, cfg.inter, true);
    l.fc2 = bind_lin(c, p + ".mlp.fc2", cfg.inter, d, true);
    m.layers.push_back(l);
  }
  m.post = bind_norm(c, v + "post_layernorm", d, cfg.eps);
  m.proj = bind_lin(c, pre + "visual_projection", d, cfg.proj, false);
  m.bound = true;
}

void finish_binding(Ctx& c, const std::string& prefix) {
  UG_CHECK(hipStreamSynchronize(c.stream));
  std::vector<std::string> unused;
  for (auto it = c.raw.begin(); it != c.raw.end();) {
    if (it->first.compare(0, prefix.size(), prefix) != 0) { ++it; continue; }
    const bool ignorable = it->first.size() >= 12 && it->first.compare(it->first.size() - 12, 12, "position_ids") == 0;
    if (!it->second.used && !ignorable) unused.push_back(it->first);
    (void)hipFree(it->second.dev);
    it = c.raw.erase(it);
  }
  if (!unused.empty()) {
    std::string s = "unexpected tensors in state dict (architecture restatement mismatch): ";
    for (size_t i = 0; i < unused.size() && i < 8; ++i) s += unused[i] + " ";
    throw std::runtime_error(s + "(" + std::to_string(unused.size()) + " total)");
  }
}

static void unfused_attention(Ctx& c, const f16* qkv, long ldqkv, int B, int S, int heads, int d, f16* out, long ldo) {
  const int Spad = pad8(S), C = heads * d;
  const size_t mk = c.ws.mark();
  float* sc = c.ws.get<float>((long)B * heads * S * Spad);
  f16* P = c.ws.get<f16>((long)B * heads * S * Spad);
  f16* Vt = c.ws.get<f16>((long)B * heads * d * Spad);
  GemmP p; memset(&p, 0, sizeof(p));
  p.A0 = qkv; p.C0 = (int)ldqkv; p.M = S; p.N = S; p.K = d; p.W = qkv + C; p.ldw = ldqkv;
  p.c0 = 1.0f / sqrtf((float)d); p.Out = sc; p.ldo = Spad; p.flags = UG_F_OUT_F32;
  p.nb_inner = heads; p.sA_o = (long)S * ldqkv; p.sA_i = d; p.sW_o = (long)S * ldqkv; p.sW_i = d;
  p.sO_o = (long)heads * S * Spad; p.sO_i = (long)S * Spad;
  run_gemm(c, p, B * heads, "gemm_attn_qk");
  {
    ProfScope ps(c, "softmax_rows", 0, (double)B * heads * S * Spad * 6.0);
    launch_softmax_rows(sc, Spad, P, Spad, (long)B * heads * S, S, c.stream);
  }
  {
    ProfScope ps(c, "transpose", 0, (double)B * heads * S * d * 4.0);
    launch_transpose(qkv + 2 * C, ldqkv, (long)S * ldqkv, Vt, Spad, (long)heads * d * Spad, B * heads, S, d, heads, d,
                     (long)d * Spad, c.stream);
  }
  GemmP q; memset(&q, 0, sizeof(q));
  q.A0 = P; q.C0 = Spad; q.M = S; q.N = d; q.K = Spad; q.W = Vt; q.ldw = Spad; q.c0 = 1.f;
  q.Out = out; q.ldo = ldo; q.nb_inner = heads;
  q.sA_o = (long)heads * S * Spad; q.sA_i = (long)S * Spad; q.sW_o = (long)heads * d * Spad; q.sW_i = (long)d * Spad;
  q.sO_o = (long)S * ldo; q.sO_i = d;
  run_gemm(c, q, B * heads, "gemm_attn_pv");
  c.ws.release(mk);
}

void test_unfused_attention(Ctx& c, const f16* qkv, long ld, int B, int S, int H, int d, f16* out, long ldo) {
  unfused_attention(c, qkv, ld, B, S, H, d, out, ldo);
}

static void res2d_forward(Ctx& c, const Res2D& r, const f16* x0, int C0, const f16* x1, int C1, int T, int h, int w,
                          int G, const f16* tproj, f16* out, StatPart* out_stats = nullptr, const StatPart* in_stats = nullptr) {
  const long M = (long)T * h * w;
  const int cin = C0 + C1, cout = r.c1.cout;
  const size_t mk = c.ws.mark();
  f16* a = c.ws.get<f16>(M * cin);
  groupnorm(c, x0, C0, x1, C1, T, h * w, G, r.n1, 0, 1, a, C1 == 0 ? in_stats : nullptr);
  f16* hb = c.ws.get<f16>(M * cout);
  StatPart sh = stat_alloc(c, M, cout, T, h * w, G, 0);
  { Epi e; e.bias2 = tproj; e.so = &sh; conv(c, a, cin, nullptr, 0, T, h, w, r.c1, 1, 1, 1, 1, hb, e); }
  f16* b = c.ws.get<f16>(M * cout);
  groupnorm(c, hb, cout, nullptr, 0, T, h * w, G, r.n2, 0, 1, b, &sh);
  const f16* res = x0;
  if (r.has_sc) {
    f16* scb = hb;
    conv(c, x0, C0, x1, C1, T, h, w, r.sc, 1, 0, 0, 1, scb);
    res = scb;
  } else {
    UG_REQUIRE(C1 == 0, "identity shortcut needs a single source");
  }
  { Epi e; e.R1 = res; e.ldr1 = cout; e.so = out_stats; conv(c, b, cout, nullptr, 0, T, h, w, r.c2, 1, 1, 1, 1, out, e); }
  c.ws.release(mk);
}

static f16* stres_forward(Ctx& c, const STRes& rb, const f16* x0, int C0, const f16* x1, int C1, int T, int h, int w,
                          int G, const f16* tproj_s, const f16* tproj_t, StatPart* out_stats = nullptr, const StatPart* in_stats = nullptr,
                          int nv = 1) {
  const long Mv = (long)T * h * w, M = nv * Mv;
  const int cout = rb.cout;
  f16* out = c.ws.get<f16>(M * cout);
  if (out_stats) *out_stats = stat_alloc(c, M, cout, nv * T, h * w, G, 0);
  const size_t mk = c.ws.mark();
  f16* xs = c.ws.get<f16>(M * cout);
  StatPart sx = stat_alloc(c, M, cout, T, h * w, G, 1), sh = stat_alloc(c, M, cout, T, h * w, G, 1);
  res2d_forward(c, rb.s, x0, C0, x1, C1, nv * T, h, w, G, tproj_s, xs, &sx, in_stats);
  auto view = [&](const StatPart& sp, int v) {
    StatPart r = sp;
    if (v > 0) { if (sp.part && sp.rb > 0 && Mv % sp.rb == 0) r.part = sp.part + v * (Mv / sp.rb) * cout; else r.rb = 0; }
    return r;
  };
  auto tconv = [&](const Conv& cv, const f16* in, f16* o, Epi e, StatPart* so) {
    if (nv == 1) { e.so = so; conv(c, in, cout, nullptr, 0, T, h, w, cv, 1, 0, 0, 1, o, e); return; }
    const f16* r1 = e.R1;
    int rb0 = 0;
    for (int v = 0; v < nv; ++v) {
      const long off = v * Mv * cout;
      StatPart sv;
      if (so && so->part) { sv.part = so->part; if (v > 0 && rb0 > 0 && Mv % rb0 == 0) sv.part += v * (Mv / rb0) * cout; }
      Epi ev = e; ev.so = (so && so->part) ? &sv : nullptr;
      if (r1) ev.R1 = r1 + off;
      conv(c, in + off, cout, nullptr, 0, T, h, w, cv, 1, 0, 0, 1, o + off, ev);
      if (v == 0) rb0 = sv.rb; else if (sv.rb != rb0) rb0 = 0;
    }
    if (so && so->part) so->rb = (rb0 > 0 && Mv % rb0 == 0) ? rb0 : 0;
  };
  f16* a = c.ws.get<f16>(M * cout);
  for (int v = 0; v < nv; ++v) { const StatPart sv = view(sx, v); groupnorm(c, xs + v * Mv * cout, cout, nullptr, 0, T, h * w, G, rb.t.n1, 1, 1, a + v * Mv * cout, &sv); }
  f16* hb = c.ws.get<f16>(M * cout);
  { Epi e; e.bias2 = tproj_t; tconv(rb.t.c1, a, hb, e, &sh); }
  for (int v = 0; v < nv; ++v) { const StatPart sv = view(sh, v); groupnorm(c, hb + v * Mv * cout, cout, nullptr, 0, T, h * w, G, rb.t.n2, 1, 1, a + v * Mv * cout, &sv); }
  { Epi e; e.c0 = 1.f - rb.alpha; e.R1 = xs; e.ldr1 = cout; e.c1 = 1.f; tconv(rb.t.c2, a, out, e, out_stats); }
  c.ws.release(mk);
  return out;
}

static bool ff_pair_fusable(const Ctx& c, long M, const Lin& f1, const Lin& f2, const Epi& e2) {
  const int C4 = f1.out / 2, C = f2.out;
  return (c.ff_fused & 1) && !c.fp8_linears && ff_fused_supported(C) && f1.in == C && C4 == 4 * C && M >= 32768 && f1.b && !e2.act && !e2.flags &&
         (!e2.R1 || !e2.ldr1 || e2.ldr1 == C) && (!e2.R2 || !e2.ldr2 || e2.ldr2 == C) && !e2.bias2;
}
struct PreNorm { const f16* g; const f16* b; float eps; const f16* addvec; long rows_per_vec; };
static long ff_fused_rows(const Ctx& c, long M) {
  const long ntile = (M + 127) / 128, full = ntile / 256 * 256, rem = ntile - full;
  static const bool nosplit = getenv("UG_FF_NOSPLIT") != nullptr;
  return (full > 0 && rem > 0 && rem <= 160 && !nosplit && !c.cosched) ? full * 128 : M;
}
static void ff_pair(Ctx& c, const f16* a, long M, const Lin& f1, const Lin& f2, f16* mid, f16* out, const Epi& e2, const QAct* q = nullptr,
                    const PreNorm* pre = nullptr, bool no_fuse = false) {
  const int C4 = f1.out / 2, C = f2.out;
  UG_REQUIRE(!pre || ff_pair_fusable(c, M, f1, f2, e2), "ff_pair: pre-norm only with the fused kernel");
  if (ff_pair_fusable(c, M, f1, f2, e2) && !no_fuse) {
    FFusedP p; memset(&p, 0, sizeof(p));
    p.X = a; p.W1 = f1.w; p.b1 = f1.b; p.W2 = f2.w; p.b2 = f2.b; p.R1 = e2.R1; p.R2 = e2.R2; p.c0 = e2.c0; p.c1 = e2.c1; p.c2 = e2.c2;
    p.Out = out; p.M = (int)M; p.C = C; p.zero = c.zero; p.variant = c.ff_variant;
    if (pre) { p.ln_g = pre->g; p.ln_b = pre->b; p.ln_eps = pre->eps; p.addvec = pre->addvec; p.rows_per_vec = (int)pre->rows_per_vec; }
    char nm[64];
    if (c.prof_on && c.prof_shapes) snprintf(nm, sizeof(nm), "gemm_ff_fused:%ldx%d", M, C); else snprintf(nm, sizeof(nm), "gemm_ff_fused");
    ProfScope ps(c, nm, 2.0 * M * (double)(2 * C4) * C + 2.0 * M * (double)C * C4,
                 2.0 * ((double)M * C * (2 + (e2.R1 ? 1 : 0) + (e2.R2 ? 1 : 0)) + 3.0 * (double)C4 * C));
    launch_ff_fused(p, c.stream);
    return;
  }
  const long bytes = M * C4 * 2;
  int nchunk = 1;
  if (bytes > (96L << 20) && getenv("UG_FF_CHUNK") && !q) nchunk = (int)((bytes + (48L << 20) - 1) / (48L << 20));
  const long rows = ((M + nchunk - 1) / nchunk + 255) / 256 * 256;
  for (long r0 = 0; r0 < M; r0 += rows) {
    const long m = std::min(rows, M - r0);
    { Epi e; e.flags = UG_F_GEGLU; if (q && nchunk == 1) { e.a8 = q->a8; e.sa8 = q->sa; e.ld_sa8 = q->ld; } linear(c, a + r0 * f1.in, m, f1, mid + r0 * C4, e); }
    Epi e = e2;
    if (e.R1) e.R1 += r0 * (e.ldr1 ? e.ldr1 : C);
    if (e.R2) e.R2 += r0 * (e.ldr2 ? e.ldr2 : C);
    linear(c, mid + r0 * C4, m, f2, out + r0 * C, e);
  }
}

static void ln_linear(Ctx& c, const f16* x, long M, const Norm& ln, f16* t1, const Lin& l, f16* out, const QAct* q) {
  layernorm(c, x, M, ln, t1, nullptr, 1, nullptr, q);
  Epi e;
  if (q) { e.a8 = q->a8; e.sa8 = q->sa; e.ld_sa8 = q->ld; }
  linear(c, t1, M, l, out, e);
}

static void ln_ff(Ctx& c, const f16* x, long M, const Norm& ln, const f16* addvec, long rows_per_vec, f16* xout, f16* t1,
                  const Lin& f1, const Lin& f2, f16* mid, f16* out, const Epi& e2, const QAct* q) {
  const int C = f2.out;
  if ((c.ff_fused & 2) && ff_pair_fusable(c, M, f1, f2, e2) && ln.g && ln.b && e2.R1 == (addvec ? xout : x) && (!addvec || xout)) {
    const long M1 = ff_fused_rows(c, M);
    Epi e = e2; e.R1 = x;
    const PreNorm pre = {ln.g, ln.b, ln.eps, addvec, rows_per_vec};
    ff_pair(c, x, M1, f1, f2, mid, out, e, nullptr, &pre);
    if (M1 < M) {
      const long o = M1 * C;
      layernorm(c, x + o, M - M1, ln, t1 + o, addvec, rows_per_vec, addvec ? xout + o : nullptr, nullptr, M1);
      Epi et = e2; et.R1 = (addvec ? xout : x) + o; if (et.R2) et.R2 += o;
      ff_pair(c, t1 + o, M - M1, f1, f2, mid, out + o, et, nullptr, nullptr, true);
    }
    return;
  }
  layernorm(c, x, M, ln, t1, addvec, rows_per_vec, xout, q);
  if (ff_pair_fusable(c, M, f1, f2, e2)) {
    const long M1 = ff_fused_rows(c, M), o = M1 * C;
    ff_pair(c, t1, M1, f1, f2, mid, out, e2, q);
    if (M1 < M) {
      Epi et = e2; if (et.R1) et.R1 += o; if (et.R2) et.R2 += o;
      ff_pair(c, t1 + o, M - M1, f1, f2, mid, out + o, et, q, nullptr, true);
    }
    return;
  }
  ff_pair(c, t1, M, f1, f2, mid, out, e2, q);
}

static f16* transformer_forward(Ctx& c, const Transformer& tr, const f16* x, int T, int h, int w, int G, const StatPart* in_stats = nullptr,
                                int nv = 1, int vid0 = 0) {
  const int C = tr.C, HW = h * w;
  const long M = (long)nv * T * HW;
  f16* out = c.ws.get<f16>(M * C);
  const size_t mk = c.ws.mark();
  f16* t1 = c.ws.get<f16>(M * C);
  groupnorm(c, x, C, nullptr, 0, nv * T, HW, G, tr.gn, 0, 0, t1, in_stats);
  f16* h0 = c.ws.get<f16>(M * C);
  const bool q8 = c.fp8_linears && !getenv("UG_NO_LNQ") && C % 128 == 0 && M >= 256 && tr.qkv1.w8 && tr.ff1.w8 && tr.ffin1.w8 && tr.tqkv.w8 && tr.tff1.w8;
  QAct qa; if (q8) qa = qact_alloc(c, M, C);
  const QAct* qp = q8 ? &qa : nullptr;
  auto qepi = [&](Epi e) { if (q8) { e.a8 = qa.a8; e.sa8 = qa.sa; e.ld_sa8 = qa.ld; } return e; };
  f16* qkv = c.ws.get<f16>(M * 3 * C);
  linear(c, t1, M, tr.proj_in, h0);
  ln_linear(c, h0, M, tr.ln1, t1, tr.qkv1, qkv, qp);
  f16* ao = c.ws.get<f16>(M * C);
  {
    FlashP p; p.Q = qkv; p.K = qkv + C; p.V = qkv + 2 * C; p.ldq = p.ldk = p.ldv = 3 * C; p.O = ao; p.ldo = C;
    p.B = nv * T; p.H = tr.heads; p.S = HW; p.scale = 0.125f; p.variant = c.flash_variant;
    char nm[96];
    if (c.prof_on && c.prof_shapes) snprintf(nm, sizeof(nm), "flash_attn:B%dxH%dxS%d", nv * T, tr.heads, HW);
    else snprintf(nm, sizeof(nm), "flash_attn");
    ProfScope ps(c, nm, 4.0 * nv * T * tr.heads * (double)HW * HW * 64, 0);
// ... 694 lines not shown
```

unigeo_amd/csrc/kernels/conv_halo.hip:

```cpp
#include "gemm_common.h"
#include <algorithm>
#include <cstdlib>
#include <type_traits>

template <int BM, int BN, int LG, bool ST = false>
__global__ __launch_bounds__(12 * 64, 3) void conv_halo_kernel(const GemmP p) {
  constexpr int BK = 64, NCW = 8, WMW = 4, WNW = 2;
  constexpr unsigned SENT = 0x80000000u;
  constexpr int WTM = BM / WMW, WTN = BN / WNW;
  constexpr int MT = WTM / 16, NT = WTN / 16;
  constexpr int WID = 4 * NT;
  constexpr int LB = BN / 32;
  constexpr int WSLOT = BN * BK;
  constexpr int TW = 1 << LG, TH = BM >> LG;
  constexpr int PITCH = (TW + 2 + 7) & ~7;
  constexpr int GPR = PITCH / 8;
  constexpr int NG = (TH + 2) * GPR;
  constexpr int HALO = NG * 8 * BK;
  constexpr int HL = 2;
  constexpr int HSLOTS = 7 * HL;
  static_assert(TH * TW == BM && TW >= 16 && (NG + 3) / 4 <= HSLOTS, "tile geometry");
  static_assert((2 * HALO + 3 * WSLOT) * 2 <= 160 * 1024, "LDS");
  extern __shared__ __attribute__((aligned(16))) f16 smem[];
  f16* halo = smem;
  f16* ring = smem + 2 * HALO;

  const int tid = threadIdx.x, lane = tid & 63;
  const int wave = __builtin_amdgcn_readfirstlane(tid >> 6);
  const bool producer = wave >= NCW;
  const int ntn = (p.N + BN - 1) / BN, ntm = p.M / BM;
  const int ntiles = ntm * ntn;
  const int Cin = p.C0 + p.C1, nchunks = Cin / BK, nk = nchunks * 9;
  const int txn = p.Wo >> LG, tpf = (p.Ho / TH) * txn;

  const int nwg = gridDim.x, w = blockIdx.x;
  const TileWalk tw = tile_walk(p.flags, ntiles, nwg, w);
  const int my_tiles = tw.count;
  const int total_it = my_tiles * nk;

  auto tile_origin = [&](int tile, int& t, int& y0, int& x0, int& n0) {
    int tm, tn; tile_coord_p(p, tile, ntm, ntn, tm, tn);
    const int tmg = tm + p.m_off / BM;
    t = tmg / tpf;
    const int rem = tmg - t * tpf;
    const int tyi = rem / txn, txi = rem - tyi * txn;
    y0 = tyi * TH; x0 = txi * TW; n0 = tn * BN;
  };

  if (producer) {
    const int pw = wave - NCW;
    const int pc = lane & 7, lrow = lane >> 3;
    const int lc16_0 = (pc ^ ((0 + (lrow >> 1)) & 7)) * 16, lc16_1 = (pc ^ ((4 + (lrow >> 1)) & 7)) * 16;
    const int lc16_h = (pc ^ (((lrow >> 1) & 3) * 2)) * 16;
    const __amdgpu_buffer_rsrc_t rA0 = __builtin_amdgcn_make_buffer_rsrc((void*)p.A0, 0, (int)SENT, 0x00020000);
    const __amdgpu_buffer_rsrc_t rA1 = __builtin_amdgcn_make_buffer_rsrc((void*)(p.A1 ? p.A1 : p.A0), 0, (int)SENT, 0x00020000);
    const __amdgpu_buffer_rsrc_t rW = __builtin_amdgcn_make_buffer_rsrc((void*)p.W, 0, (int)SENT, 0x00020000);
    constexpr int ngw_max = (NG + 3) / 4;
    const int ngw = (NG - pw + 3) >> 2;
    int h_pix[HSLOTS];
    auto halo_setup = [&](int tile) {
      int t, y0, x0, n0; tile_origin(tile, t, y0, x0, n0);
#pragma unroll
      for (int k = 0; k < ngw_max; ++k) {
        const int grp = pw + 4 * k;
        const int hy = grp / GPR, hx = (grp - hy * GPR) * 8 + lrow;
        const int y = y0 - 1 + hy, x = x0 - 1 + hx;
        const bool ok = grp < NG && hx < TW + 2 && y >= 0 && y < p.Hi && x >= 0 && x < p.Wi;
        h_pix[k] = ok ? (t * p.Hi + y) * p.Wi + x : -1;
      }
    };
    auto halo_issue = [&](int k, int chunk, int hb) {
      const int cb = chunk * BK;
      const bool src0 = cb < p.C0;
      const int Cs2 = (src0 ? p.C0 : p.C1) * 2;
      const int soff = (src0 ? cb : cb - p.C0) * 2;
      const unsigned voff = h_pix[k] >= 0 ? (unsigned)h_pix[k] * (unsigned)Cs2 + (unsigned)lc16_h : SENT;
      __builtin_amdgcn_raw_ptr_buffer_load_lds(src0 ? rA0 : rA1, (lptr_t)(halo + hb * HALO + (pw + 4 * k) * 8 * BK), 16, (int)voff, soff, 0, 0);
    };
    unsigned b_off[LB];
    int ld_ti = 0, ld_ks = 0, ld_slot = 0;
    int ld_gc = 0;
    int h_tile = -1;
    auto issue = [&]() -> int {
      if (ld_ks == 0) {
        int t, y0, x0, n0; tile_origin(tw.first + ld_ti * tw.step, t, y0, x0, n0);
#pragma unroll
        for (int l = 0; l < LB; ++l) {
          const int rg = pw * LB + l;
          const int lr = rg * 8 + lrow;
          const int part = lr / WTN, rem = lr % WTN;
          const int jj = rem >> 4, i = rem & 15;
          const int n = n0 + part * WTN + (i >> 2) * WID + jj * 4 + (i & 3);
          b_off[l] = n < p.N ? (unsigned)n * (unsigned)(p.ldw * 2) + ((rg & 1) ? lc16_1 : lc16_0) : SENT;
        }
      }
      f16* Bs = ring + ld_slot * WSLOT;
      const int kt2 = ld_ks * BK * 2;
#pragma unroll
      for (int l = 0; l < LB; ++l)
        __builtin_amdgcn_raw_ptr_buffer_load_lds(rW, (lptr_t)(Bs + (pw * LB + l) * 8 * BK), 16, (int)b_off[l], kt2, 0, 0);
      int nh = 0;
      const int chunk = ld_ks / 9, sp = ld_ks - chunk * 9;
      if (sp >= 2) {
        int tchunk = chunk + 1, ttile = ld_ti;
        if (tchunk == nchunks) { tchunk = 0; ++ttile; }
        if (ttile < my_tiles) {
          if (ttile != h_tile) { halo_setup(tw.first + ttile * tw.step); h_tile = ttile; }
#pragma unroll
          for (int u = 0; u < HL; ++u) {
            const int k = (sp - 2) * HL + u;
            if (k < ngw) {
#pragma unroll
              for (int kk = 0; kk < ngw_max; ++kk) if (kk == k) halo_issue(kk, tchunk, (ld_gc + 1) & 1);
              ++nh;
            }
          }
        }
      }
      if (++ld_ks == nk) { ld_ks = 0; ++ld_ti; }
      if (ld_ks % 9 == 0) ++ld_gc;
      if (++ld_slot == 3) ld_slot = 0;
      return nh;
    };
    if (total_it > 0) {
      halo_setup(tw.first); h_tile = 0;
#pragma unroll
      for (int k = 0; k < ngw_max; ++k) if (k < ngw) halo_issue(k, 0, 0);
      issue();
    }
    if (total_it > 1) issue();
    if (total_it > 1) asm volatile("s_waitcnt vmcnt(%0)" ::"n"(LB) : "memory");
    else asm volatile("s_waitcnt vmcnt(0)" ::: "memory");
    __builtin_amdgcn_s_barrier();
    for (int fi = 0; fi < total_it; ++fi) {
      if (fi + 2 < total_it) {
        const int nh = issue();
        if (nh == 2) asm volatile("s_waitcnt vmcnt(%0)" ::"n"(LB + 2) : "memory");
        else if (nh == 1) asm volatile("s_waitcnt vmcnt(%0)" ::"n"(LB + 1) : "memory");
        else asm volatile("s_waitcnt vmcnt(%0)" ::"n"(LB) : "memory");
      } else {
        asm volatile("s_waitcnt vmcnt(0)" ::: "memory");
      }
      __builtin_amdgcn_s_barrier();
    }
    return;
  }

  const int wm = wave / WNW, wn = wave % WNW;
  f32x4 acc[MT][NT];
#pragma unroll
  for (int i = 0; i < MT; ++i)
#pragma unroll
    for (int j = 0; j < NT; ++j) acc[i][j] = (f32x4){0.f, 0.f, 0.f, 0.f};
  const int l15 = lane & 15, g = lane >> 4;
  const int sw = swz<BK>(l15);
  const int r0 = wm * WTM;
  const int hpb = (r0 >> LG) * PITCH + (r0 & (TW - 1)) + l15;
  auto DI = [](int i) constexpr { return TW >= 64 ? i * 16 : TW == 32 ? (i >> 1) * PITCH + (i & 1) * 16 : i * PITCH; };
  static_assert(TW >= 64 || (TW == 32 && WTM % 32 == 0) || TW == 16, "row-block offsets");
  int a_pre[3][2], b_pre[2];
#pragma unroll
  for (int dx = 0; dx < 3; ++dx)
#pragma unroll
    for (int kk = 0; kk < 2; ++kk) {
      const int hp = hpb + dx;
      a_pre[dx][kk] = (hp * BK + (((kk * 4 + g) ^ (((hp >> 1) & 3) * 2)) * 8)) * 2;
    }
#pragma unroll
  for (int kk = 0; kk < 2; ++kk) b_pre[kk] = ((wn * WTN + l15) * BK + (((kk * 4 + g) ^ sw) * 8)) * 2;
  const char* ringb = (const char*)ring;
  int cp_ti = 0, cp_gc = 0;
  __builtin_amdgcn_s_barrier();
  asm volatile("" ::: "memory");
  const char* Hb = nullptr;
  int ti = 0;
  bool last_chunk = false;
  const bool lean = !ST && BN != 160 && tile_epilogue_lean_ok(p, WTN, true) && !(p.tune_knobs & 8388608);
  auto step = [&](auto TAP) {
    constexpr int tap = decltype(TAP)::value;
    constexpr int dy = tap / 3, dx = tap - dy * 3;
    constexpr int slot = tap % 3;
    {
      f16x8 af[2][MT], bf[2][NT];
#pragma unroll
      for (int kk = 0; kk < 2; ++kk) {
#pragma unroll
        for (int j = 0; j < NT; ++j) bf[kk][j] = *(const f16x8*)(ringb + b_pre[kk] + (slot * WSLOT + j * 16 * BK) * 2);
#pragma unroll
        for (int i = 0; i < MT; ++i) af[kk][i] = *(const f16x8*)(Hb + a_pre[dx][kk] + (dy * PITCH + DI(i)) * BK * 2);
      }
#pragma unroll
      for (int kk = 0; kk < 2; ++kk)
#pragma unroll
        for (int i = 0; i < MT; ++i)
#pragma unroll
          for (int j = 0; j < NT; ++j)
            acc[i][j] = __builtin_amdgcn_mfma_f32_16x16x32_f16(bf[kk][j], af[kk][i], acc[i][j], 0, 0, 0);
      constexpr int R = MT + NT, Q = MT * NT;
      __builtin_amdgcn_sched_group_barrier(0x100, R, 0);
#pragma unroll
      for (int r = 0; r < R; ++r) {
        __builtin_amdgcn_sched_group_barrier(0x008, Q / R, 0);
        __builtin_amdgcn_sched_group_barrier(0x100, 1, 0);
      }
      __builtin_amdgcn_sched_group_barrier(0x008, Q - R * (Q / R), 0);
      __builtin_amdgcn_sched_group_barrier(0x008, Q, 0);
    }
    asm volatile("s_waitcnt lgkmcnt(0)" ::: "memory");
    __builtin_amdgcn_s_barrier();
    asm volatile("" ::: "memory");
    if (tap == 8 && last_chunk) {
      int t, y0, x0, n0; tile_origin(tw.first + ti * tw.step, t, y0, x0, n0);
      const int m0 = (t * p.Ho + y0) * p.Wo + x0 - p.m_off;
      if constexpr (ST) tile_epilogue_stats<MT, NT, WTM, WTN>(p, acc, m0, n0, wm, wn, lane, (t * tpf + (y0 / TH) * txn + (x0 >> LG)) * (BM / WTM) + wm);
      else if constexpr (BN != 160) { if (lean) tile_epilogue_lean<MT, NT, WTM, WTN, false, true>(p, acc, m0, n0, wm, wn, lane, 0, nullptr); else tile_epilogue<MT, NT, WTM, WTN>(p, acc, m0, n0, wm, wn, lane, 0); }
      else tile_epilogue<MT, NT, WTM, WTN>(p, acc, m0, n0, wm, wn, lane, 0);
    }
  };
  for (ti = 0; ti < my_tiles; ++ti) {
    for (int c = 0; c < nchunks; ++c, ++cp_gc) {
      Hb = (const char*)(halo + (cp_gc & 1) * HALO);
      last_chunk = c == nchunks - 1;
      step(std::integral_constant<int, 0>{}); step(std::integral_constant<int, 1>{}); step(std::integral_constant<int, 2>{});
      step(std::integral_constant<int, 3>{}); step(std::integral_constant<int, 4>{}); step(std::integral_constant<int, 5>{});
      step(std::integral_constant<int, 6>{}); step(std::integral_constant<int, 7>{}); step(std::integral_constant<int, 8>{});
    }
  }
  (void)cp_ti;
}

static bool halo_geom_ok(const GemmP& p, int bm, int lg) {
  const int tw = 1 << lg, th = bm >> lg;
  if (th < 1 || th * tw != bm || p.Wo % tw || p.Ho % th) return false;
  const long band = (long)th * p.Wo;
  return p.m_off % band == 0 && p.M % band == 0;
}
static int halo_pick_lg(const GemmP& p, int bm, int bn) {
  if (bm == 256 && bn == 160) return halo_geom_ok(p, 256, 5) ? 5 : -1;
  if (bm == 256) { for (int lg : {4, 5, 6}) if (halo_geom_ok(p, 256, lg)) return lg; return -1; }
  return halo_geom_ok(p, 192, 4) ? 4 : -1;
}

bool conv_halo_supported(const GemmP& p, int batch, int bm, int bn) {
  if (!p.conv || batch != 1 || p.kt != 1 || p.ky != 3 || p.kx != 3 || p.stride != 1 || p.ups != 1 || p.pad_t != 1 || p.pad_l != 1) return false;
  if (!p.kchunk || p.up_phase || p.splitk > 1 || p.Hi != p.Ho || p.Wi != p.Wo) return false;
  const int Cin = p.C0 + p.C1;
  if (Cin % 64 || p.C0 % 64 || p.M % bm || p.m_off % bm || p.N % 16) return false;
  const long lim = (1L << 31) - 64;
  if ((long)p.T * p.Hi * p.Wi * std::max(p.C0, p.C1) * 2 >= lim || (long)p.N * p.ldw * 2 >= lim) return false;
  if (p.m_off == 0 && p.M != p.T * p.Ho * p.Wo) return false;
  return halo_pick_lg(p, bm, bn) >= 0;
}

template <int BM, int BN, int LG, bool ST = false>
static void launch_halo_t(const GemmP& p, hipStream_t s) {
  constexpr int TW = 1 << LG, TH = BM >> LG, PITCH = (TW + 2 + 7) & ~7, NG = (TH + 2) * (PITCH / 8);
  const size_t lds = 2 * (size_t)NG * 1024 + 3 * (size_t)BN * 128;
  static bool attr[32] = {};
  bool& at = attr[ug_dev_slot()];
  if (!at) {
    UG_CHECK(hipFuncSetAttribute((const void*)conv_halo_kernel<BM, BN, LG, ST>, hipFuncAttributeMaxDynamicSharedMemorySize, 160 * 1024));
    at = true;
  }
  const int ntiles = (p.M / BM) * cdiv(p.N, BN);
  int gx = std::min(256, ntiles);
  static const bool dbg = getenv("UG_HALO_DEBUG") != nullptr;
  if (dbg) fprintf(stderr, "[halo] %dx%d M %d (m_off %d) N %d C %d+%d  %dx%d  tile %dx%d pitch %d  lds %zu  grid %d\n", BM, BN, p.M, p.m_off, p.N, p.C0, p.C1, p.Ho, p.Wo, TH, TW, PITCH, lds, gx);
  GemmP q = p; q.halo_lg = LG; q.halo_tw = TW; q.splitk = 1;
  hipLaunchKernelGGL((conv_halo_kernel<BM, BN, LG, ST>), dim3(gx), dim3(12 * 64), lds, s, q);
}

void launch_conv_halo(const GemmP& p, int bm, int bn, hipStream_t s) {
  const int lg = halo_pick_lg(p, bm, bn);
  UG_REQUIRE(lg >= 0, "halo conv: no tile geometry");
  if (p.stat_part) {
    UG_REQUIRE(bn == 128, "halo conv: epilogue statistics on 128-column tiles only");
    if (bm == 192) launch_halo_t<192, 128, 4, true>(p, s);
    else if (lg == 4) launch_halo_t<256, 128, 4, true>(p, s); else if (lg == 5) launch_halo_t<256, 128, 5, true>(p, s); else launch_halo_t<256, 128, 6, true>(p, s);
    return;
  }
  if (bm == 256 && bn == 160) launch_halo_t<256, 160, 5>(p, s);
  else if (bm == 256) { if (lg == 4) launch_halo_t<256, 128, 4>(p, s); else if (lg == 5) launch_halo_t<256, 128, 5>(p, s); else launch_halo_t<256, 128, 6>(p, s); }
  else if (bn == 160) launch_halo_t<192, 160, 4>(p, s);
  else launch_halo_t<192, 128, 4>(p, s);
}
```

unigeo_amd/csrc/kernels/gemm.hip:

```cpp
#include "../common.h"
#include <algorithm>

#include "gemm_common.h"

template <int BM, int BN, int BK, int NST, int WMW, int WNW> struct GemmOcc {
  static constexpr int lds = NST * (BM + BN) * BK * 2;
  static constexpr int wg_lds = (160 * 1024) / lds;
  static constexpr int wg = wg_lds < 1 ? 1 : (wg_lds > 4 ? 4 : wg_lds);
  static constexpr int wps_raw = wg * WMW * WNW / 4;
  static constexpr int wps = wps_raw < 1 ? 1 : (wps_raw > 4 ? 4 : wps_raw);
};

#ifdef UG_GEMM_TRACE
#define UG_STAMP(slot)                                                                                   \
  do {                                                                                                   \
    if (traced && fi >= 8 && fi < 32) {                                                                  \
      unsigned long long c_;                                                                             \
      asm volatile("s_memtime %0\n\ts_waitcnt lgkmcnt(0)" : "=s"(c_)::"memory");                         \
      if (lane == 0) tr_lds[(fi - 8) * 5 + (slot)] = (unsigned)c_;                                       \
    }                                                                                                    \
  } while (0)
#else
#define UG_STAMP(slot) do {} while (0)
#endif
// ... 1089 lines not shown
    const int ntm = cdiv(p.M, bm), ntn = cdiv(p.N, bn);
    int g = 1;
    if (!(p.tune_knobs & 32) && (double)p.N * p.K * 2.0 > 3.0 * (1 << 20) && ntm >= 2 && ntn >= 2)
      while (g * 2 <= ntm && (double)(g * 2) * (g * 2) <= 32.0 * percu * bn / bm * 1.5) g *= 2;
    p.group_m = g;
  }
  switch (pick) {
    case 0: launch_mx<256, 256, 2, 2, 4>(p, s); break;
    case 1: launch_mx<256, 128, 3, 4, 2>(p, s); break;
    case 3: launch_mx<192, 128, 3, 4, 2>(p, s); break;
    default: launch_mx<128, 128, 2, 2, 2>(p, s); break;
  }
  UG_CHECK(hipGetLastError());
}





struct TileCand { int id, bm, bn, percu; float dense, conv; bool geglu_ok; };
static const TileCand kCands[] = {
    {15, 256, 256, 1, 1200.f, 1190.f, true},  {35, 256, 256, 1, 1190.f, 1200.f, true},  {59, 256, 128, 1, 1143.f, 1154.f, false},
    {54, 256, 128, 1, 1135.f, 1150.f, true},  {19, 256, 128, 1, 1044.f, 1002.f, false}, {0, 128, 128, 2, 890.f, 1025.f, true},
    {14, 256, 64, 2, 880.f, 883.f, false},    {1, 128, 64, 3, 757.f, 799.f, false},    {12, 64, 64, 5, 456.f, 652.f, false},
    {63, 192, 128, 1, 1030.f, 1120.f, false}, {64, 192, 128, 1, 1020.f, 1110.f, true}};

void gemm_plan(const GemmP& p, int batch, int* cfg_out, int* split_out) {
  const bool geglu = p.flags & UG_F_GEGLU;
  int cfg = 15;
  float best = -1.f;
  for (const TileCand& c : kCands) {
    if (geglu && !c.geglu_ok) continue;
    const long tm = cdiv(p.M, c.bm), tn = cdiv(p.N, c.bn);
    const long tiles = tm * tn * batch, slots = (long)c.percu * 256;
    const float fill = (p.tune_knobs & 4194304) ? 1.f : (float)tiles / (cdiv(tiles, slots) * slots);
    float sc = (p.conv ? c.conv : c.dense) * ((float)p.M / (tm * c.bm)) * ((float)p.N / (tn * c.bn)) * fill;
    if (c.id == 19 && p.conv && p.K <= 512) sc *= 1.25f;
    if ((c.id == 15 || c.id == 35) && !p.conv && !geglu && p.K <= 384) sc *= 0.9f;
    if (sc > best) { best = sc; cfg = c.id; }
  }
  if (!p.conv && !geglu && p.M >= 50000 && p.N > 256 && p.N <= 384 && p.K >= 1024) cfg = 4;
  if (!(p.tune_knobs & 4096) && batch == 1) {
    const bool bufa = gemm_can_bufa(p, 64, true);
    if (!p.conv && geglu && p.M >= 4096 && p.N >= 4096 && p.K >= 512) cfg = bufa ? 35 : 15;
    else if (!p.conv && geglu && p.K <= 384 && p.M < 32768 && p.M >= 4096) cfg = (p.tune_knobs & 16777216) ? 64 : (bufa ? 35 : 15);
    else if (!p.conv && !geglu && cfg == 63 && p.K >= 2048 && p.N <= 1280) cfg = 64;
    else if (!p.conv && !geglu && p.M >= 50000 && p.K <= 384 && p.N >= 640 && p.N < 2048 && bufa) cfg = 59;
    else if (!p.conv && !geglu && p.N <= 384 && p.K >= 1024 && p.M > 2048 && p.M <= 16384) cfg = 3;
    else if (p.conv && p.kt > 1 && p.N > 256 && p.N <= 320 && p.M >= 50000 && !(p.tune_knobs & 524288)) cfg = 14;
  }
  int split = 1;
  const long tiles128 = (long)cdiv(p.M, 128) * cdiv(p.N, 128) * batch;
  const int nk = cdiv(p.K, 64);
  const bool plain_epi = !geglu && !p.up_phase && !(p.flags & UG_F_OUT_F32) && batch == 1 && (p.N % 8 == 0) && (p.ldo % 8 == 0) &&
                         (!p.R1 || p.ldr1 % 8 == 0) && (!p.R2 || p.ldr2 % 8 == 0);
  if (!geglu && p.M <= 2048 && p.N < 2048) {
    cfg = 3;
    if (plain_epi && p.N >= 128) {
      if (nk >= 128) {
        for (int sp = 8; sp >= 2; --sp)
          if ((512 / sp) >= tiles128 && nk / sp >= 16) { split = sp; cfg = 0; break; }
      }
      if (split == 1 && nk >= 48) split = 2;
    }
    if (plain_epi && p.N >= 128) {
      const long t64 = (long)cdiv(p.M, 128) * cdiv(p.N, 64);
      if (p.conv && tiles128 <= 64 && nk >= 64) {
        int sp = (int)std::min<long>(std::min<long>(512 / tiles128, nk / 7), 24);
        while (sp >= 2 && (512 / sp) < tiles128) --sp;
        if (sp >= 2) { cfg = 0; split = sp; }
      } else if (!p.conv && t64 <= 64 && nk >= 16) {
        const int sp = (int)std::min<long>(256 / t64, nk / 5);
        if (sp >= 2) { cfg = 3; split = sp; }
      }
    }
    if (!(p.tune_knobs & 8192) && plain_epi && p.N >= 128) {
      const long t192 = (long)cdiv(p.M, 192) * cdiv(p.N, 128), t64b = (long)cdiv(p.M, 128) * cdiv(p.N, 64);
      if (p.conv && p.M > 128 && t192 <= 128 && nk >= 16 && gemm_can_bufa(p, 64, true)) {
        cfg = 63; split = (int)std::max<long>(1, std::min<long>(std::min<long>(160 / t192, nk / 8), 8));
      } else if (p.conv && p.M <= 128 && nk >= 64) {
        const int sp = (int)std::min<long>(std::min<long>(240 / t64b, nk / 7), 24);
        if (sp >= 2) { cfg = 3; split = sp; }
      } else if (!p.conv && split == 1 && nk >= 32 && t64b <= 128 && t64b > 64) split = 2;
    }
    if (!(p.tune_knobs & 2048) && plain_epi && p.M > 1024 && p.N >= 1024 && p.N < 2048 && gemm_can_bufa(p, 64, true)) {
      if (p.conv && nk >= 128) { cfg = 59; split = 4; }
      else if (p.conv && nk >= 48) { cfg = 63; split = 3; }
      else if (!p.conv && nk >= 64) { cfg = 59; split = 3; }
    }
  } else if (!(p.tune_knobs & 512) && plain_epi && p.M <= 8192 && tiles128 <= 256 && p.N >= 128 && p.N < 2048 && (p.conv ? nk >= 32 : nk >= 16)) {
    const long t192u = (long)cdiv(p.M, 192) * cdiv(p.N, 128);
    if (p.conv && !(p.tune_knobs & 8192) && t192u <= 128 && gemm_can_bufa(p, 64, true)) {
      cfg = 63; split = (int)std::max<long>(1, std::min<long>(std::min<long>(160 / t192u, nk / 8), 8));
    } else if (p.conv) {
      int sp = (int)std::min<long>(std::min<long>(512 / tiles128, nk / 8), 8);
      while (sp >= 2 && (512 / sp) < tiles128) --sp;
      cfg = 0; split = std::max(1, sp);
    } else {
      const long t64 = (long)cdiv(p.M, 128) * cdiv(p.N, 64);
      cfg = 3;
      const int sp = (int)std::min<long>(std::min<long>(512 / t64, nk / 8), 8);
      split = std::max(1, sp);
      if (!(p.tune_knobs & 8192) && t64 > 128) split = 1;
    }
  } else if (!geglu && !p.conv && p.M <= 512 && p.N >= 2048) {
    cfg = 3;
  } else if (!(p.tune_knobs & 8192) && !geglu && !p.conv && batch == 1 && p.M <= 8192 && p.K <= 384 && p.N <= 384) {
    cfg = 3;
  }
  if ((p.tune_cfg_p1 - 1) >= 0 && !(geglu && (p.tune_cfg_p1 - 1) != 0 && (p.tune_cfg_p1 - 1) != 4 && (p.tune_cfg_p1 - 1) != 8 && (p.tune_cfg_p1 - 1) != 15 && (p.tune_cfg_p1 - 1) != 35 && (p.tune_cfg_p1 - 1) != 54 && (p.tune_cfg_p1 - 1) != 62 && (p.tune_cfg_p1 - 1) != 64)) cfg = (p.tune_cfg_p1 - 1);
  if ((p.tune_split_p1 - 1) >= 0) split = plain_epi ? std::max(1, (p.tune_split_p1 - 1)) : 1;
  *cfg_out = cfg; *split_out = split;
}

static int pick_group_m(const GemmP& p, int cfg, int batch, int split) {
  if ((p.conv && (p.tune_knobs & 64)) || batch > 1 || (p.tune_knobs & 32)) return 1;
  if ((double)p.N * p.K * 2.0 <= 3.0 * (1 << 20)) return 1;
  int bm = 256, bn = 128, percu = 1;
  switch (cfg) {
    case 0: bm = 128; bn = 128; percu = 2; break;
    case 1: case 3: bm = 128; bn = 64; percu = cfg == 1 ? 3 : 2; break;
    case 12: bm = 64; bn = 64; percu = 5; break;
    case 14: case 34: bm = 256; bn = 64; percu = 2; break;
    case 15: case 35: bm = 256; bn = 256; break;
    case 60: case 70: bm = 256; bn = 160; break;
    case 61: case 62: case 63: case 64: case 72: bm = 192; bn = 128; break;
    case 73: bm = 192; bn = 160; break;
    default: break;
  }
  const int ntm = cdiv(p.M, bm), ntn = cdiv(p.N, bn);
  if (ntm < 2 || ntn < 2) return 1;
  const double P = 32.0 * percu;
  int g = 1;
  while (g * 2 <= ntm && (double)(g * 2) * (g * 2) <= P * bn / bm * 1.5) g *= 2;
  if (!(p.tune_knobs & 1048576) && (double)g * ntn <= P) g = 1;
  return g;
}

static bool cfg_geom(int cfg, int& bm, int& bn, int& wmw, int& wnw) {
  switch (cfg) {
    case 0: bm = 128; bn = 128; wmw = 2; wnw = 2; return true;
    case 1: case 3: bm = 128; bn = 64; wmw = 2; wnw = 2; return true;
    case 4: case 8: case 54: bm = 256; bn = 128; wmw = 4; wnw = 2; return true;
    case 12: bm = 64; bn = 64; wmw = 2; wnw = 2; return true;
    case 14: case 34: bm = 256; bn = 64; wmw = 4; wnw = 2; return true;
    case 15: case 35: bm = 256; bn = 256; wmw = 2; wnw = 4; return true;
    case 19: case 39: case 59: bm = 256; bn = 128; wmw = 2; wnw = 4; return true;
    case 61: case 63: bm = 192; bn = 128; wmw = 2; wnw = 4; return true;
    case 62: case 64: bm = 192; bn = 128; wmw = 4; wnw = 2; return true;
    default: return false;
  }
}

void launch_gemm(const GemmP& p0, int batch, hipStream_t s, int* stat_rb) {
  GemmP p = p0;
  if (stat_rb) *stat_rb = 0;
  if (!stat_rb) p.stat_part = nullptr;
  if (p.tune_knobs & 2) p.flags |= UG_F_NOXCD;
  if (p.tune_knobs & 128) p.flags |= UG_F_XCDROUND;
  if (p.tune_knobs & 16) p.flags |= UG_F_PRIO;
  UG_REQUIRE(p.K % 8 == 0, "GEMM K must be a multiple of 8");
  UG_REQUIRE(p.ldw % 8 == 0, "GEMM ldw must be a multiple of 8");
  UG_REQUIRE(p.M > 0 && p.N > 0 && p.K > 0, "empty GEMM");
  UG_REQUIRE(p.zero != nullptr, "zero page missing");
  UG_REQUIRE(p.nb_inner >= 1, "nb_inner");
  if (p.flags & UG_F_GEGLU) UG_REQUIRE(p.N % 128 == 0, "GEGLU GEMM needs N % 128 == 0");
  if (p.conv) {
    UG_REQUIRE(p.C0 % 8 == 0 && p.C1 % 8 == 0, "conv channel counts must be multiples of 8");
    UG_REQUIRE(p.K == (p.C0 + p.C1) * p.kt * p.ky * p.kx, "conv K mismatch");
    UG_REQUIRE(p.M == p.T * p.Ho * p.Wo && p.m_off == 0, "conv M mismatch");
    UG_REQUIRE(p.ups == 1 || p.ups == 2, "ups");
  } else {
    UG_REQUIRE(p.C0 % 8 == 0, "dense lda must be a multiple of 8");
  }
  int cfg = p.cfg_p1 - 1, split = p.splitk;
  if (cfg < 0 || split < 1) { int c2, s2; gemm_plan(p, batch, &c2, &s2); if (cfg < 0) cfg = c2; if (split < 1) split = s2; }
  if (p.flags & UG_F_GEGLU) UG_REQUIRE(cfg == 0 || cfg == 4 || cfg == 8 || cfg == 15 || cfg == 35 || cfg == 54 || cfg == 62 || cfg == 64, "GEGLU needs a 64-column wave tile");
  p.splitk = split;
  bool planned = p0.cfg_p1 == 0;
  if (!planned && (p.tune_cfg_p1 - 1) < 0) { int c2, s2; gemm_plan(p0, batch, &c2, &s2); planned = (c2 == cfg && s2 == split); }
  const bool halo_on = planned && !(p.tune_knobs & 16384) && split == 1 && (p.tune_cfg_p1 - 1) < 0 && !(p.flags & UG_F_GEGLU);
  const bool halo_l0 = halo_on && p.N % 160 == 0 && p.N <= 320 && p.C1 == 0 && !(p.tune_knobs & 32768) && conv_halo_supported(p, batch, 256, 128);
  if (!halo_l0 && planned && p.conv && p.kt == 1 && p.ky == 3 && p.kx == 3 && p.N % 160 == 0 && p.N <= 320 && split == 1 && batch == 1 && !p.up_phase && !(p.flags & (UG_F_OUT_F32 | UG_F_GEGLU)) &&
      (p.tune_cfg_p1 - 1) < 0 && !(p.tune_knobs & 1024) && gemm_can_bufa(p, 64, true)) {
    const long ntn = p.N / 160, tiles = (long)cdiv(p.M, 256) * ntn, whole = tiles / 256 * 256, rem = tiles - whole;
    if (whole > 0 && rem > 0 && rem * 2 <= 256) {
      const int M1 = (int)(whole / ntn) * 256;
      const bool halo = false;
      GemmP a = p; a.M = M1; a.cfg_p1 = 61;
      a.stat_part = nullptr;
      GemmP b = p0; b.stat_part = nullptr; b.M = p.M - M1; b.m_off = M1; b.Out = (void*)((f16*)p.Out + (long)M1 * p.ldo);
      b.flags |= p.flags & (UG_F_NOXCD | UG_F_XCDROUND);
      if (b.R1) b.R1 += (long)M1 * p.ldr1;
      if (b.R2) b.R2 += (long)M1 * p.ldr2;
      int cb, sb; gemm_plan(b, 1, &cb, &sb);
      if (cb != 59 && cb != 60 && cb != 63 && cb != 64 && cb != 54) cb = 63;
      b.cfg_p1 = cb + 1; b.splitk = 1;
      a.splitk = 1;
      a.group_m = pick_group_m(a, 60, 1, 1); a.tm_T = a.tm_nb = 0;
      launch_cfg(halo && conv_halo_supported(a, 1, 256, 160) ? 70 : 60, a, 1, s);
      if (halo && conv_halo_supported(b, 1, 256, 160)) cb = 70;
      b.group_m = pick_group_m(b, cb, 1, 1); b.tm_T = b.tm_nb = 0;
      launch_cfg(cb, b, 1, s);
      UG_CHECK(hipGetLastError());
      return;
    }
  }
  if (halo_on) {
    int best = -1; double bfill = 0.0;
    for (int c = 70; c <= 73; ++c) {
      const int bm = c <= 71 ? 256 : 192, bn = (c == 70 || c == 73) ? 160 : 128;
      if (!conv_halo_supported(p, batch, bm, bn)) continue;
      const long tiles = (long)(p.M / bm) * cdiv(p.N, bn);
      const double useful = (double)p.N / (cdiv(p.N, bn) * bn);
      const double fill = (double)tiles / (cdiv(tiles, 256) * 256.0) * useful * (bm == 256 ? 1.0 : 0.97);
      if (fill > bfill) { bfill = fill; best = c; }
    }
    if (halo_l0) best = 71;
    else if (p.N % 160 == 0 && p.N <= 320) best = -1;
    if (best >= 0) cfg = best;
  }
  if (planned && !(p.tune_knobs & 65536) && (p.tune_cfg_p1 - 1) < 0 && split == 1 && gemm_stream_supported(p, batch)) {
    cfg = 80;
  }
  if (split > 1) UG_REQUIRE(p.partial != nullptr, "split-K needs a partial buffer");
  p.group_m = pick_group_m(p, cfg, batch, split);
  p.tm_T = p.tm_nb = 0;
  if (p.conv && p.kt > 1 && p.T > 1 && batch == 1 && !(p.tune_knobs & 256)) {
    int bm = 256;
    switch (cfg) { case 0: case 1: case 3: bm = 128; break; case 12: bm = 64; break; case 61: case 62: case 63: case 64: bm = 192; break; default: break; }
    const long hw = (long)p.Ho * p.Wo;
    if (hw % bm == 0 && hw / bm >= 1) { p.tm_T = p.T; p.tm_nb = (int)(hw / bm); }
  }
  if (p.stat_part) {
    int bm = 0, wmw = 0;
    {
      int gbm, gbn, gwm, gwn;
      const bool sym = (cfg == 14 || cfg == 19) && p.conv && gemm_can_bufa(p, 64, false) && !(p.tune_knobs & 4);
      const bool pk = (cfg == 35 || cfg == 54 || cfg == 59 || cfg == 63 || cfg == 64) && p.conv && gemm_can_bufa(p, 64, true);
      if (cfg == 71) { bm = 256; wmw = 4; }
      else if (cfg == 72) { bm = 192; wmw = 4; }
      else if ((sym || pk) && cfg_geom(cfg, gbm, gbn, gwm, gwn)) { bm = gbm; wmw = gwm; }
    }
    const int wtm = bm ? bm / wmw : 0;
    const bool ok = bm && split == 1 && batch == 1 && !(p.flags & (UG_F_GEGLU | UG_F_OUT_F32 | UG_F_R1_F32)) && !p.up_phase && !(p.tune_knobs & 131072) &&
                    p.M % bm == 0 && p.m_off == 0 && p.stat_hw > 0 && p.stat_hw % wtm == 0 && p.N % 16 == 0 && p.ldo % 8 == 0 &&
                    (!p.R1 || p.ldr1 % 8 == 0) && (!p.R2 || p.ldr2 % 8 == 0);
    static const bool sdbg = getenv("UG_STAT_DEBUG") != nullptr;
    if (sdbg) fprintf(stderr, "[stat] M %d N %d K %d conv %d kt %d hw %d cfg %d split %d -> rb %d\n", p.M, p.N, p.K, p.conv, p.kt, p.stat_hw, cfg, split, ok ? wtm : 0);
    if (ok) *stat_rb = wtm; else p.stat_part = nullptr;
  }
  launch_cfg(cfg, p, batch, s);
  if (split > 1) {
    const long nvec = (long)p.M * (p.N / 8);
    int grid = (int)std::min<long>((nvec + 255) / 256, 256 * 8);
    hipLaunchKernelGGL(splitk_epilogue, dim3(grid), dim3(256), 0, s, p);
  }
  UG_CHECK(hipGetLastError());
}
```

unigeo_amd/pipeline.py:

```python
import dataclasses
from types import SimpleNamespace

import numpy as np

from . import weights as W
from ._lib import Engine


def make_noise(T, H, W_, seed=0):
    import torch
    g = torch.Generator(device="cpu").manual_seed(int(seed))
    aug = torch.randn((T, 3, H, W_), generator=g, dtype=torch.float32)
    lat = torch.randn((1, T, 4, H // 8, W_ // 8), generator=g, dtype=torch.float32)
    return lat.numpy(), aug.numpy()


class DepthCrafterPipelineHIP:

    def __init__(self, engine, unet_cfg, vae_cfg, clip_cfg):
        self.engine, self.unet_cfg, self.vae_cfg, self.clip_cfg = engine, unet_cfg, vae_cfg, clip_cfg
        self.seed = 0
        self.decode_chunk_size = 8

    @classmethod
    def from_state(cls, unet_state, vae_state, clip_state, cfgs=None, device_id=0,
                   workspace_bytes=None, persist_bytes=None):
        u, v, c = cfgs or (W.UNetCfg(), W.VAECfg(), W.CLIPCfg())
        nbytes = sum(int(np.prod(a.shape)) * 2 for s in (unet_state, vae_state, clip_state) for a in s.values())
        eng = Engine(device_id,
                     workspace_bytes if workspace_bytes is not None else (24 << 30),
                     persist_bytes if persist_bytes is not None else int(nbytes * 1.35) + (256 << 20))
        eng.load_state("unet.", unet_state); eng.bind_unet(u)
        eng.load_state("vae.", vae_state); eng.bind_vae(v)
        eng.load_state("clip.", clip_state); eng.bind_clip(c)
        return cls(eng, u, v, c)

    @classmethod
    def from_pretrained(cls, pre_train_path, unet_path, device_id=0, **kw):
        u, v, c, cfgs = W.load_pretrained(unet_path, pre_train_path, with_cfgs=True)
        return cls.from_state(u, v, c, cfgs=cfgs, device_id=device_id, **kw)

    @classmethod
    def from_random(cls, seed=42, cfgs=None, device_id=0, **kw):
        u, v, c = cfgs or (W.UNetCfg(), W.VAECfg(), W.CLIPCfg())
        return cls.from_state(W.random_state(W.unet_manifest(u), seed),
                              W.random_state(W.vae_manifest(v), seed + 1),
                              W.random_state(W.clip_manifest(c), seed + 2), cfgs=(u, v, c), device_id=device_id, **kw)

    def to(self, device):
        return self

    def enable_xformers_memory_efficient_attention(self):
        return None

    def enable_attention_slicing(self):
        return None

    def __call__(self, video, height=None, width=None, num_inference_steps=25, guidance_scale=1.0,
                 window_size=110, noise_aug_strength=0.02, decode_chunk_size=None, output_type="np",
                 overlap=25, track_time=False, noise_latents=None, noise_aug=None, seed=None,
                 intrinsics=None, with_normals=False, return_frames=True, noise="host"):
        if noise not in ("host", "device"):
            raise ValueError('noise must be "host" or "device"')
        if noise == "device" and (noise_latents is not None or noise_aug is not None):
            raise ValueError('noise="device" generates the noise from the seed: do not pass noise_latents / noise_aug')
        u8 = getattr(video, "dtype", None) == np.uint8
        if u8:
            video = np.asarray(video)
            if video.ndim != 4 or video.shape[1] != 3:
                raise ValueError("uint8 video must be planar [T,3,H,W]")
            T, _, H, Wd = video.shape
        else:
            video = np.asarray(video, dtype=np.float32)
            if video.ndim != 4 or video.shape[-1] != 3:
                raise ValueError("video must be [T,H,W,3] float in [0,1]")
            T, H, Wd, _ = video.shape
        if (height not in (None, H)) or (width not in (None, Wd)):
            raise ValueError("height/width must equal the frame size (the reference passes frames.shape)")
        if H % 64 or Wd % 64:
            raise ValueError("height and width must be multiples of 64")
        guidance_scale = float(guidance_scale)
        if not np.isfinite(guidance_scale):
            raise ValueError("guidance_scale must be finite")
        if T > window_size and window_size > 128:
            raise ValueError("a denoising window holds at most 128 frames (temporal attention tile); pass window_size <= 128")
        if T > window_size and not 0 <= overlap < window_size:
            raise ValueError("overlap must be in [0, window_size)")
        if abs(noise_aug_strength - 0.02) > 1e-9:
            raise NotImplementedError("noise_aug_strength is fixed at the pipeline default 0.02")
        if output_type != "np":
            raise NotImplementedError('only output_type="np" (what the reference requests)')
        seed = self.seed if seed is None else seed
        if noise == "device":
            if not 0 <= int(seed) < 1 << 64:
                raise ValueError("the noise seed must be in [0, 2**64)")
        elif noise_latents is None or noise_aug is None:
            noise_latents, noise_aug = make_noise(T, H, Wd, seed)
        chunk = decode_chunk_size or self.decode_chunk_size
        eng = self.engine
        if noise == "device":
            eng.set_inputs_ex(video, seed=int(seed), intrinsics=intrinsics)
        elif u8:
            eng.set_inputs_ex(video, noise_latents=noise_latents, noise_aug=noise_aug, intrinsics=intrinsics)
        else:
            eng.set_inputs(video, noise_latents, noise_aug, intrinsics)
        eng.set_guidance(guidance_scale)
        eng.run(num_inference_steps, chunk, with_normals=with_normals, window=window_size if T > window_size else 0, overlap=overlap)
        frames, depth, normals = eng.get_outputs(frames=bool(return_frames), depth=True, normals=with_normals)
        return SimpleNamespace(frames=[frames], depth=depth, normals=normals)
```

unigeo_amd/stablenormal.py:

```python
import math
import os

import numpy as np

from . import weights as W
from ._lib import Engine

PROMPT = "The normal map"


def refine_timesteps(start=401, steps=10):
    return [int(round(start - i * start / steps)) for i in range(steps)]


def ddim_tables(timesteps, prediction_type="v_prediction", num_train=1000, beta_start=0.00085, beta_end=0.012):
    betas = np.linspace(beta_start ** 0.5, beta_end ** 0.5, num_train, dtype=np.float64) ** 2
    ab = np.cumprod(1.0 - betas)
    ca, cb = [], []
    for i, t in enumerate(timesteps):
        at = ab[int(t)]
        ap = ab[int(timesteps[i + 1])] if i + 1 < len(timesteps) else 1.0
        sa, s1, pa, p1 = math.sqrt(at), math.sqrt(1 - at), math.sqrt(ap), math.sqrt(1 - ap)
        if prediction_type == "epsilon":
            a, b = pa / sa, p1 - pa * s1 / sa
        elif prediction_type == "v_prediction":
            a, b = pa * sa + p1 * s1, p1 * sa - pa * s1
        elif prediction_type == "sample":
            a, b = p1 / s1, pa - p1 * sa / s1
        else:
            raise ValueError(f"unknown prediction_type {prediction_type!r}")
        ca.append(a); cb.append(b)
    return np.asarray(ca, np.float32), np.asarray(cb, np.float32)


def normals_to_uint8(n):
    return (np.clip((np.asarray(n, np.float32) + 1.0) * 0.5, 0.0, 1.0) * 255.0).astype(np.uint8)


COMPONENTS = ("vae", "unet_yoso", "controlnet_yoso", "unet", "controlnet_dino", "dino")


def manifests(cfgs):
    u, v, d = cfgs
    return {"vae": W.sd_vae_manifest(v), "unet_yoso": W.sd_unet_manifest(u), "controlnet_yoso": W.controlnet_manifest(u),
            "unet": W.sd_unet_manifest(u), "controlnet_dino": W.controlnet_manifest(u, d.hidden_size), "dino": W.dino_manifest(d)}


class StableNormalPredictorHIP:

    parity = "unpinned"

    def __init__(self, engine, cfgs, prompt_embeds, yoso_timestep=999, refine_start=401, refine_steps=10, prediction_type="v_prediction",
                 processing_resolution=0):
        self.engine, self.cfgs = engine, cfgs
        self.processing_resolution = int(processing_resolution)
        self.prediction_type = prediction_type
        try:
            engine.set_concurrency(2)
        except AttributeError:
            pass
        self.prompt_embeds = np.ascontiguousarray(prompt_embeds, dtype=np.float32)
        if self.prompt_embeds.shape != (77, cfgs[0].cross_attention_dim):
            raise ValueError(f"prompt_embeds must be [77, {cfgs[0].cross_attention_dim}]")
        self.yoso_timestep = float(yoso_timestep)
        self.timesteps = refine_timesteps(refine_start, refine_steps) if refine_steps > 0 else []
        self.ca, self.cb = ddim_tables(self.timesteps, prediction_type) if self.timesteps else (np.zeros(0, np.float32), np.zeros(0, np.float32))

    @classmethod
    def from_states(cls, states, cfgs=None, prompt_embeds=None, device_id=0, workspace_bytes=None, persist_bytes=None, **kw):
        cfgs = cfgs or (W.SDUNetCfg(), W.VAECfg(), W.DinoCfg())
        nbytes = sum(int(np.prod(a.shape)) * 2 for s in states.values() for a in s.values())
        eng = Engine(device_id, workspace_bytes if workspace_bytes is not None else (24 << 30),
                     persist_bytes if persist_bytes is not None else int(nbytes * 1.2) + (256 << 20))
        for comp in COMPONENTS:
            eng.load_state(f"sn.{comp}.", states[comp])
        eng.bind_stablenormal(*cfgs)
        return cls(eng, cfgs, prompt_embeds, **kw)

    @classmethod
    def from_random(cls, seed=7, cfgs=None, **kw):
        cfgs = cfgs or (W.SDUNetCfg(), W.VAECfg(), W.DinoCfg())
        ms = manifests(cfgs)
        states = {c: W.random_state(ms[c], seed + i) for i, c in enumerate(COMPONENTS)}
        pe = np.random.default_rng(seed + 100).standard_normal((77, cfgs[0].cross_attention_dim)).astype(np.float16).astype(np.float32)
        return cls.from_states(states, cfgs, prompt_embeds=pe, **kw)

    @classmethod
    def from_pretrained(cls, model_dir, cfgs=None, **kw):
        states, pe = W.load_stablenormal_pretrained(model_dir, cfgs)
        return cls.from_states(states, cfgs, prompt_embeds=pe, **kw)

    def predict_batch(self, images01):
        x = np.ascontiguousarray(images01, dtype=np.float32)
        if x.ndim != 4 or x.shape[-1] != 3:
            raise ValueError("images must be [B,H,W,3] float in [0,1]")
        H, Wd = x.shape[1:3]
        R = self.processing_resolution
        if R > 0:
            sc = R / float(max(H, Wd))
            ph, pw = max(64, int(round(H * sc / 64.0)) * 64), max(64, int(round(Wd * sc / 64.0)) * 64)
            if (ph, pw) != (H, Wd):
                n = self.engine.sn_run(self.engine.resize_bilinear(x, ph, pw), self.prompt_embeds, self.yoso_timestep, self.timesteps, self.ca, self.cb)
                return self.engine.resize_bilinear(n, H, Wd, normalise=True)
        if H % 64 or Wd % 64:
            raise ValueError("height and width must be multiples of 64 (or set processing_resolution)")
        return self.engine.sn_run(x, self.prompt_embeds, self.yoso_timestep, self.timesteps, self.ca, self.cb)

    def __call__(self, image):
        from PIL import Image
        a = np.asarray(image)
        n = self.predict_batch(a[None].astype(np.float32) / 255.0)[0]
        return Image.fromarray(normals_to_uint8(n))
```

Before: 28.64 frames/s.

## Fold resnet 1x1 shortcut conv into the 3x3 conv2 halo GEMM

```diff
diff --git a/unigeo_amd/_lib.py b/unigeo_amd/_lib.py
--- a/unigeo_amd/_lib.py
+++ b/unigeo_amd/_lib.py
@@ -14,7 +14,7 @@
     "ug_load_tensor", "ug_bind_unet", "ug_bind_vae", "ug_bind_clip",
     "ug_dc_set_inputs", "ug_dc_run", "ug_dc_run_windows", "ug_dc_get_outputs", "ug_dc_device_ptrs", "ug_dc_set_trace", "ug_dc_set_guidance", "ug_unet_forward_pair", "ug_dc_set_inputs_ex", "ug_dc_get_noise", "ug_op_philox_u32", "ug_op_randn", "ug_op_u8_to_frames", "ug_set_vae_encode_fp32", "ug_set_concurrency", "ug_set_coscheduled", "ug_set_fp8_linears", "ug_op_linear_mx8", "ug_set_ff_fused", "ug_op_ff", "ug_op_ln_ff", "ug_bench_ff", "ug_bench_flash", "ug_tune_flash", "ug_tune_ff",
     "ug_eval_depth", "ug_eval_normal", "ug_depth_eval_opts_default", "ug_eval_depth_ex", "ug_eval_depth_global", "ug_op_masked_median", "ug_clip_embed", "ug_vae_encode", "ug_vae_decode", "ug_unet_forward", "ug_normals_from_depth",
-    "ug_op_linear", "ug_op_conv", "ug_op_conv_gn", "ug_op_groupnorm", "ug_op_layernorm", "ug_op_flash_attn",
+    "ug_op_linear", "ug_op_conv", "ug_op_conv_gn", "ug_op_conv_fold", "ug_op_groupnorm", "ug_op_layernorm", "ug_op_flash_attn",
     "ug_op_temporal_attn", "ug_op_attention_generic", "ug_op_flash_attn_dh", "ug_op_euler_step", "ug_op_flash_cross_attn", "ug_op_temporal_attn_nv",
     "ug_op_split_pair", "ug_op_gn32_pair", "ug_op_conv_wide", "ug_op_attn_wide",
     "ug_bind_stablenormal", "ug_sn_run", "ug_sn_unet_forward", "ug_sn_dino", "ug_sn_vae_decode", "ug_sn_vae_encode", "ug_resize_bilinear",
@@ -154,6 +154,7 @@
     lib.ug_op_conv.argtypes = [vp, vp, ip, vp, ip, ip, ip, ip, vp, vp, ip, ip, ip, ip, ip, ip, ip, vp]
     lib.ug_op_groupnorm.argtypes = [vp, vp, ip, vp, ip, ip, ip, ip, C.c_float, ip, ip, vp, vp, vp]
     lib.ug_op_conv_gn.argtypes = [vp, vp, ip, ip, ip, ip, vp, vp, vp, ip, ip, ip, ip, C.c_float, ip, vp, vp, vp, vp, vp, vp]
+    lib.ug_op_conv_fold.argtypes = [vp, vp, ip, vp, ip, vp, ip, ip, ip, ip, vp, vp, vp, vp, ip, ip, ip, vp, vp, vp]
     lib.ug_op_layernorm.argtypes = [vp, vp, ip, ip, C.c_float, vp, vp, vp, ip, vp, vp]
     lib.ug_op_flash_attn.argtypes = [vp, vp, ip, ip, ip, vp]
     lib.ug_op_temporal_attn.argtypes = [vp, vp, ip, ip, ip, vp]
@@ -862,6 +863,17 @@
                                         _ptr(_f32(gamma)), _ptr(_f32(beta)), _ptr(co), _ptr(y1), _ptr(y2), C.byref(rb)))
         return co, y1, y2, rb.value
 
+    def op_conv_fold(self, b, x0, x1, w3, bias3, wsc, bias_sc, cfg=-1, stats=False):
+        b = _f32(b); T, H, W, Cc = b.shape; x0 = _f32(x0); x1a = None if x1 is None else _f32(x1)
+        w3 = _f32(w3); O = w3.shape[0]; wsc = _f32(wsc)
+        SC0 = x0.shape[-1]; SC1 = 0 if x1a is None else x1a.shape[-1]
+        assert wsc.shape == (O, SC0 + SC1) and w3.shape == (O, Cc, 3, 3)
+        o1 = np.empty((T, H, W, O), np.float32); o2 = np.empty_like(o1)
+        info = (C.c_int * 2)(0, 0)
+        self._ck(self.lib.ug_op_conv_fold(self.ctx, _ptr(b), Cc, _ptr(x0), SC0, _ptr(x1a), SC1, T, H, W, _ptr(w3), _ptr(_f32(bias3)), _ptr(wsc), _ptr(_f32(bias_sc)),
+                                          O, int(cfg), int(bool(stats)), _ptr(o1), _ptr(o2), info))
+        return o1, o2, info[0], info[1]
+
     def op_layernorm(self, x, eps, gamma, beta, addvec=None, rows_per_vec=1):
         x = _f32(x); M, Cc = x.shape
         out = np.empty((M, Cc), np.float32); xout = np.empty((M, Cc), np.float32)
diff --git a/unigeo_amd/csrc/common.h b/unigeo_amd/csrc/common.h
--- a/unigeo_amd/csrc/common.h
+++ b/unigeo_amd/csrc/common.h
@@ -67,6 +67,7 @@
   int halo_tw, halo_lg;
   int tune_cfg_p1, tune_split_p1, tune_knobs;
   float2* stat_part; int stat_hw;
+  const f16* S0; const f16* S1; int SC0, SC1;
 };
 struct GemmTune { int cfg = -1, split = -1, knobs = 0; };
 static inline void gemm_apply_tune(GemmP& p, const GemmTune& t) { p.tune_cfg_p1 = t.cfg + 1; p.tune_split_p1 = t.split + 1; p.tune_knobs = t.knobs; }
@@ -77,6 +78,8 @@
 void launch_gemm_stream(const GemmP& p, hipStream_t s);
 bool conv_halo_supported(const GemmP& p, int batch, int bm, int bn);
 void launch_conv_halo(const GemmP& p, int bm, int bn, hipStream_t s);
+bool conv_fold_pays(const GemmP& p);
+int conv_fold_cfg(const GemmP& p, int batch, int split);
 void gemm_plan(const GemmP& p, int batch, int* cfg_out, int* split_out);
 
 struct FFusedP {
diff --git a/unigeo_amd/csrc/engine.h b/unigeo_amd/csrc/engine.h
--- a/unigeo_amd/csrc/engine.h
+++ b/unigeo_amd/csrc/engine.h
@@ -33,7 +33,8 @@
              const unsigned char* w8 = nullptr; const unsigned* sw8 = nullptr; long ld_sw8 = 0; };
 struct Conv { const f16* w = nullptr; const f16* b = nullptr; int cin = 0, cinp = 0, cout = 0, kt = 1, ky = 1, kx = 1;
               const f16* wphase = nullptr;
-              int kchunk = 0; };
+              int kchunk = 0;
+              const f16* wfold = nullptr; int fold_c = 0; };
 struct Norm { const f16* g = nullptr; const f16* b = nullptr; int c = 0; float eps = 1e-5f; };
 
 struct Res2D { Norm n1, n2; Conv c1, c2, sc; Lin temb; bool has_sc = false, has_temb = false; int tidx = -1; };
diff --git a/unigeo_amd/csrc/engine.hip b/unigeo_amd/csrc/engine.hip
--- a/unigeo_amd/csrc/engine.hip
+++ b/unigeo_amd/csrc/engine.hip
@@ -524,6 +524,14 @@
   r.n2 = bind_norm(c, p + ".norm2", cout, eps);
   r.c2 = bind_conv(c, p + ".conv2", cout, cout, 1, 3);
   if (cin != cout) { r.sc = bind_conv(c, p + ".conv_shortcut", cin, cout, 1, 1); r.has_sc = true; }
+  if (r.has_sc && r.c2.kchunk && cin % 64 == 0 && r.c2.b && r.sc.b) {
+    const long k3 = 9L * cout, ld = k3 + cin;
+    f16* wf = c.persist.get<f16>((long)cout * ld);
+    launch_copy2d(r.c2.w, k3, wf, ld, cout, (int)k3, c.stream);
+    launch_copy2d(r.sc.w, cin, wf + k3, ld, cout, cin, c.stream);
+    UG_CHECK(hipStreamSynchronize(c.stream));
+    r.c2.wfold = wf; r.c2.fold_c = cin;
+  }
   return r;
 }
 static ResT bind_rest(Ctx& c, const std::string& p, int ch, int temb, float eps) {
@@ -829,6 +837,20 @@
   f16* b = c.ws.get<f16>(M * cout);
   groupnorm(c, hb, cout, nullptr, 0, T, h * w, G, r.n2, 0, 1, b, &sh);
   const f16* res = x0;
+  if (r.has_sc && r.c2.wfold && C0 % 64 == 0 && C1 % 64 == 0 && C0 + C1 == r.c2.fold_c) {
+    GemmP p; memset(&p, 0, sizeof(p));
+    p.conv = 1; p.A0 = b; p.C0 = cout; p.T = T; p.Hi = p.Ho = h; p.Wi = p.Wo = w; p.ups = 1; p.stride = 1; p.pad_t = 1; p.pad_l = 1; p.kt = 1; p.ky = 3; p.kx = 3;
+    p.M = (int)M; p.N = cout; p.K = 9 * cout; p.W = r.c2.wfold; p.ldw = p.K + r.c2.fold_c; p.bias = r.c2.b; p.bias2 = r.sc.b;
+    p.c0 = 1.f; p.c1 = 1.f; p.c2 = 1.f; p.Out = out; p.ldo = cout; p.ldr1 = p.ldr2 = cout; p.kchunk = 1;
+    p.S0 = x0; p.SC0 = C0; p.S1 = x1; p.SC1 = C1;
+    GemmP q = p; q.zero = c.zero; q.nb_inner = 1; gemm_apply_tune(q, c.tune);
+    int cf, sp; gemm_plan(q, 1, &cf, &sp);
+    if (conv_fold_cfg(q, 1, sp) >= 0 && conv_fold_pays(q)) {
+      run_gemm(c, p, 1, "gemm_conv3x3_sc", 1.f, out_stats);
+      c.ws.release(mk);
+      return;
+    }
+  }
   if (r.has_sc) {
     f16* scb = hb;
     conv(c, x0, C0, x1, C1, T, h, w, r.sc, 1, 0, 0, 1, scb);
diff --git a/unigeo_amd/csrc/kernels/conv_halo.hip b/unigeo_amd/csrc/kernels/conv_halo.hip
--- a/unigeo_amd/csrc/kernels/conv_halo.hip
+++ b/unigeo_amd/csrc/kernels/conv_halo.hip
@@ -3,7 +3,7 @@
 #include <cstdlib>
 #include <type_traits>
 
-template <int BM, int BN, int LG, bool ST = false>
+template <int BM, int BN, int LG, bool ST = false, bool SC = false>
 __global__ __launch_bounds__(12 * 64, 3) void conv_halo_kernel(const GemmP p) {
   constexpr int BK = 64, NCW = 8, WMW = 4, WNW = 2;
   constexpr unsigned SENT = 0x80000000u;
@@ -21,6 +21,7 @@
   constexpr int HSLOTS = 7 * HL;
   static_assert(TH * TW == BM && TW >= 16 && (NG + 3) / 4 <= HSLOTS, "tile geometry");
   static_assert((2 * HALO + 3 * WSLOT) * 2 <= 160 * 1024, "LDS");
+  static_assert(LB + HL <= 63 && HL == 2, "the fetch waves' counted waits: vmcnt(LB + slices issued), slices in {0, 1, 2}");
   extern __shared__ __attribute__((aligned(16))) f16 smem[];
   f16* halo = smem;
   f16* ring = smem + 2 * HALO;
@@ -30,7 +31,9 @@
   const bool producer = wave >= NCW;
   const int ntn = (p.N + BN - 1) / BN, ntm = p.M / BM;
   const int ntiles = ntm * ntn;
-  const int Cin = p.C0 + p.C1, nchunks = Cin / BK, nk = nchunks * 9;
+  const int Cin = p.C0 + p.C1, nchunks = Cin / BK;
+  const int nsc = SC ? (p.SC0 + p.SC1) / BK : 0;
+  const int nk = nchunks * 9 + (nsc + 2) / 3 * 3;
   const int txn = p.Wo >> LG, tpf = (p.Ho / TH) * txn;
 
   const int nwg = gridDim.x, w = blockIdx.x;
@@ -79,6 +82,98 @@
     };
     unsigned b_off[LB];
     int ld_ti = 0, ld_ks = 0, ld_slot = 0;
+    if constexpr (SC) {
+      const __amdgpu_buffer_rsrc_t rS0 = __builtin_amdgcn_make_buffer_rsrc((void*)p.S0, 0, (int)SENT, 0x00020000);
+      const __amdgpu_buffer_rsrc_t rS1 = __builtin_amdgcn_make_buffer_rsrc((void*)(p.S1 ? p.S1 : p.S0), 0, (int)SENT, 0x00020000);
+      const int n9 = nchunks * 9, ipt = nchunks + nsc;
+      unsigned h_in = 0;
+#pragma unroll
+      for (int k = 0; k < ngw_max; ++k) {
+        const int grp = pw + 4 * k;
+        const int hy = grp / GPR, hx = (grp - hy * GPR) * 8 + lrow;
+        if (grp < NG && hy >= 1 && hy <= TH && hx >= 1 && hx <= TW) h_in |= 1u << k;
+      }
+      auto sc_issue = [&](int k, int j, int hb) {
+        const int cb = j * BK;
+        const bool src0 = cb < p.SC0;
+        const int Cs2 = (src0 ? p.SC0 : p.SC1) * 2;
+        const int soff = (src0 ? cb : cb - p.SC0) * 2;
+        const unsigned voff = ((h_in >> k) & 1) ? (unsigned)h_pix[k] * (unsigned)Cs2 + (unsigned)lc16_h : SENT;
+        __builtin_amdgcn_raw_ptr_buffer_load_lds(src0 ? rS0 : rS1, (lptr_t)(halo + hb * HALO + (pw + 4 * k) * 8 * BK), 16, (int)voff, soff, 0, 0);
+      };
+      auto issue = [&]() -> int {
+        int nh = 0;
+        if (ld_ks == 0) {
+          int t, y0, x0, n0; tile_origin(tw.first + ld_ti * tw.step, t, y0, x0, n0);
+#pragma unroll
+          for (int l = 0; l < LB; ++l) {
+            const int rg = pw * LB + l;
+            const int lr = rg * 8 + lrow;
+            const int part = lr / WTN, rem = lr % WTN;
+            const int jj = rem >> 4, i = rem & 15;
+            const int n = n0 + part * WTN + (i >> 2) * WID + jj * 4 + (i & 3);
+            b_off[l] = n < p.N ? (unsigned)n * (unsigned)(p.ldw * 2) + ((rg & 1) ? lc16_1 : lc16_0) : SENT;
+          }
+        }
+        if (ld_ks < n9 + nsc) {
+          f16* Bs = ring + ld_slot * WSLOT;
+          const int kt2 = ld_ks * BK * 2;
+#pragma unroll
+          for (int l = 0; l < LB; ++l)
+            __builtin_amdgcn_raw_ptr_buffer_load_lds(rW, (lptr_t)(Bs + (pw * LB + l) * 8 * BK), 16, (int)b_off[l], kt2, 0, 0);
+          if (ld_ks < n9) {
+            const int chunk = ld_ks / 9, sp = ld_ks - chunk * 9;
+            if (sp >= 2) {
+              const int hb = (ld_ti * ipt + chunk + 1) & 1;
+#pragma unroll
+              for (int u = 0; u < HL; ++u) {
+                const int k = (sp - 2) * HL + u;
+                if (k < ngw) {
+#pragma unroll
+                  for (int kk = 0; kk < ngw_max; ++kk) if (kk == k) { if (chunk + 1 < nchunks) halo_issue(kk, chunk + 1, hb); else sc_issue(kk, 0, hb); }
+                  ++nh;
+                }
+              }
+            }
+          }
+        } else nh = -1;
+        if (++ld_ks == nk) { ld_ks = 0; ++ld_ti; }
+        if (++ld_slot == 3) ld_slot = 0;
+        return nh;
+      };
+      auto late_image = [&](int ti, int ks) {
+        if (ks == 0) {
+          halo_setup(tw.first + ti * tw.step);
+#pragma unroll
+          for (int k = 0; k < ngw_max; ++k) if (k < ngw) halo_issue(k, 0, (ti * ipt) & 1);
+        } else if (ks > n9 && ks < n9 + nsc) {
+#pragma unroll
+          for (int k = 0; k < ngw_max; ++k) if (k < ngw) sc_issue(k, ks - n9, (ti * ipt + nchunks + ks - n9) & 1);
+        }
+      };
+      halo_setup(tw.first);
+#pragma unroll
+      for (int k = 0; k < ngw_max; ++k) if (k < ngw) halo_issue(k, 0, 0);
+      issue(); issue();
+      asm volatile("s_waitcnt vmcnt(%0)" ::"n"(LB) : "memory");
+      __builtin_amdgcn_s_barrier();
+      int nx_ti = 0, nx_ks = 1;
+      for (int fi = 0; fi < total_it; ++fi) {
+        if (fi + 1 < total_it) late_image(nx_ti, nx_ks);
+        if (++nx_ks == nk) { nx_ks = 0; ++nx_ti; }
+        if (fi + 2 < total_it) {
+          const int nh = issue();
+          if (nh == 2) asm volatile("s_waitcnt vmcnt(%0)" ::"n"(LB + 2) : "memory");
+          else if (nh == 1) asm volatile("s_waitcnt vmcnt(%0)" ::"n"(LB + 1) : "memory");
+          else if (nh == 0) asm volatile("s_waitcnt vmcnt(%0)" ::"n"(LB) : "memory");
+          else asm volatile("s_waitcnt vmcnt(0)" ::: "memory");
+        } else {
+          asm volatile("s_waitcnt vmcnt(0)" ::: "memory");
+        }
+        __builtin_amdgcn_s_barrier();
+      }
+      return;
+    }
     int ld_gc = 0;
     int h_tile = -1;
     auto issue = [&]() -> int {
@@ -176,10 +271,9 @@
   int ti = 0;
   bool last_chunk = false;
   const bool lean = !ST && BN != 160 && tile_epilogue_lean_ok(p, WTN, true) && !(p.tune_knobs & 8388608);
-  auto step = [&](auto TAP) {
-    constexpr int tap = decltype(TAP)::value;
+  auto mma = [&](auto TAP, auto SLOT) {
+    constexpr int tap = decltype(TAP)::value, slot = decltype(SLOT)::value;
     constexpr int dy = tap / 3, dx = tap - dy * 3;
-    constexpr int slot = tap % 3;
     {
       f16x8 af[2][MT], bf[2][NT];
 #pragma unroll
@@ -207,15 +301,29 @@
       __builtin_amdgcn_sched_group_barrier(0x008, Q, 0);
     }
     asm volatile("s_waitcnt lgkmcnt(0)" ::: "memory");
+  };
+  auto epilogue = [&]() {
+    int t, y0, x0, n0; tile_origin(tw.first + ti * tw.step, t, y0, x0, n0);
+    const int m0 = (t * p.Ho + y0) * p.Wo + x0 - p.m_off;
+    if constexpr (ST) tile_epilogue_stats<MT, NT, WTM, WTN>(p, acc, m0, n0, wm, wn, lane, (t * tpf + (y0 / TH) * txn + (x0 >> LG)) * (BM / WTM) + wm);
+    else if constexpr (BN != 160) { if (lean) tile_epilogue_lean<MT, NT, WTM, WTN, false, true>(p, acc, m0, n0, wm, wn, lane, 0, nullptr); else tile_epilogue<MT, NT, WTM, WTN>(p, acc, m0, n0, wm, wn, lane, 0); }
+    else tile_epilogue<MT, NT, WTM, WTN>(p, acc, m0, n0, wm, wn, lane, 0);
+  };
+  auto step = [&](auto TAP) {
+    constexpr int tap = decltype(TAP)::value;
+    mma(TAP, std::integral_constant<int, tap % 3>{});
     __builtin_amdgcn_s_barrier();
     asm volatile("" ::: "memory");
-    if (tap == 8 && last_chunk) {
-      int t, y0, x0, n0; tile_origin(tw.first + ti * tw.step, t, y0, x0, n0);
-      const int m0 = (t * p.Ho + y0) * p.Wo + x0 - p.m_off;
-      if constexpr (ST) tile_epilogue_stats<MT, NT, WTM, WTN>(p, acc, m0, n0, wm, wn, lane, (t * tpf + (y0 / TH) * txn + (x0 >> LG)) * (BM / WTM) + wm);
-      else if constexpr (BN != 160) { if (lean) tile_epilogue_lean<MT, NT, WTM, WTN, false, true>(p, acc, m0, n0, wm, wn, lane, 0, nullptr); else tile_epilogue<MT, NT, WTM, WTN>(p, acc, m0, n0, wm, wn, lane, 0); }
-      else tile_epilogue<MT, NT, WTM, WTN>(p, acc, m0, n0, wm, wn, lane, 0);
-    }
+    if constexpr (!SC)
+      if (tap == 8 && last_chunk) epilogue();
+  };
+  auto sc_step = [&](auto SLOT, bool live) {
+    if (live) {
+      Hb = (const char*)(halo + (cp_gc & 1) * HALO); ++cp_gc;
+      mma(std::integral_constant<int, 4>{}, SLOT);
+    }
+    __builtin_amdgcn_s_barrier();
+    asm volatile("" ::: "memory");
   };
   for (ti = 0; ti < my_tiles; ++ti) {
     for (int c = 0; c < nchunks; ++c, ++cp_gc) {
@@ -225,6 +333,14 @@
       step(std::integral_constant<int, 3>{}); step(std::integral_constant<int, 4>{}); step(std::integral_constant<int, 5>{});
       step(std::integral_constant<int, 6>{}); step(std::integral_constant<int, 7>{}); step(std::integral_constant<int, 8>{});
     }
+    if constexpr (SC) {
+      for (int j = 0; j < nsc; j += 3) {
+        sc_step(std::integral_constant<int, 0>{}, true);
+        sc_step(std::integral_constant<int, 1>{}, j + 1 < nsc);
+        sc_step(std::integral_constant<int, 2>{}, j + 2 < nsc);
+      }
+      epilogue();
+    }
   }
   (void)cp_ti;
 }
@@ -249,17 +365,21 @@
   const long lim = (1L << 31) - 64;
   if ((long)p.T * p.Hi * p.Wi * std::max(p.C0, p.C1) * 2 >= lim || (long)p.N * p.ldw * 2 >= lim) return false;
   if (p.m_off == 0 && p.M != p.T * p.Ho * p.Wo) return false;
+  if (p.S0) {
+    if (bn != 128 || p.SC0 <= 0 || p.SC0 % 64 || p.SC1 < 0 || p.SC1 % 64 || (p.SC1 > 0 && !p.S1)) return false;
+    if (p.ldw != (long)p.K + p.SC0 + p.SC1 || (long)p.T * p.Hi * p.Wi * std::max(p.SC0, p.SC1) * 2 >= lim) return false;
+  }
   return halo_pick_lg(p, bm, bn) >= 0;
 }
 
-template <int BM, int BN, int LG, bool ST = false>
+template <int BM, int BN, int LG, bool ST = false, bool SC = false>
 static void launch_halo_t(const GemmP& p, hipStream_t s) {
   constexpr int TW = 1 << LG, TH = BM >> LG, PITCH = (TW + 2 + 7) & ~7, NG = (TH + 2) * (PITCH / 8);
   const size_t lds = 2 * (size_t)NG * 1024 + 3 * (size_t)BN * 128;
   static bool attr[32] = {};
   bool& at = attr[ug_dev_slot()];
   if (!at) {
-    UG_CHECK(hipFuncSetAttribute((const void*)conv_halo_kernel<BM, BN, LG, ST>, hipFuncAttributeMaxDynamicSharedMemorySize, 160 * 1024));
+    UG_CHECK(hipFuncSetAttribute((const void*)conv_halo_kernel<BM, BN, LG, ST, SC>, hipFuncAttributeMaxDynamicSharedMemorySize, 160 * 1024));
     at = true;
   }
   const int ntiles = (p.M / BM) * cdiv(p.N, BN);
@@ -267,12 +387,23 @@
   static const bool dbg = getenv("UG_HALO_DEBUG") != nullptr;
   if (dbg) fprintf(stderr, "[halo] %dx%d M %d (m_off %d) N %d C %d+%d  %dx%d  tile %dx%d pitch %d  lds %zu  grid %d\n", BM, BN, p.M, p.m_off, p.N, p.C0, p.C1, p.Ho, p.Wo, TH, TW, PITCH, lds, gx);
   GemmP q = p; q.halo_lg = LG; q.halo_tw = TW; q.splitk = 1;
-  hipLaunchKernelGGL((conv_halo_kernel<BM, BN, LG, ST>), dim3(gx), dim3(12 * 64), lds, s, q);
+  hipLaunchKernelGGL((conv_halo_kernel<BM, BN, LG, ST, SC>), dim3(gx), dim3(12 * 64), lds, s, q);
 }
 
 void launch_conv_halo(const GemmP& p, int bm, int bn, hipStream_t s) {
   const int lg = halo_pick_lg(p, bm, bn);
   UG_REQUIRE(lg >= 0, "halo conv: no tile geometry");
+  if (p.S0) {
+    UG_REQUIRE(bn == 128, "halo conv: the folded shortcut is instantiated for 128-column tiles only");
+    if (p.stat_part) {
+      if (bm == 192) launch_halo_t<192, 128, 4, true, true>(p, s);
+      else if (lg == 4) launch_halo_t<256, 128, 4, true, true>(p, s); else if (lg == 5) launch_halo_t<256, 128, 5, true, true>(p, s); else launch_halo_t<256, 128, 6, true, true>(p, s);
+    } else {
+      if (bm == 192) launch_halo_t<192, 128, 4, false, true>(p, s);
+      else if (lg == 4) launch_halo_t<256, 128, 4, false, true>(p, s); else if (lg == 5) launch_halo_t<256, 128, 5, false, true>(p, s); else launch_halo_t<256, 128, 6, false, true>(p, s);
+    }
+    return;
+  }
   if (p.stat_part) {
     UG_REQUIRE(bn == 128, "halo conv: epilogue statistics on 128-column tiles only");
     if (bm == 192) launch_halo_t<192, 128, 4, true>(p, s);
diff --git a/unigeo_amd/csrc/kernels/gemm.hip b/unigeo_amd/csrc/kernels/gemm.hip
--- a/unigeo_amd/csrc/kernels/gemm.hip
+++ b/unigeo_amd/csrc/kernels/gemm.hip
@@ -1265,6 +1265,24 @@
   }
 }
 
+int conv_fold_cfg(const GemmP& p, int batch, int split) {
+  if (!p.S0 || (p.tune_knobs & (16384 | 33554432)) || split != 1 || (p.tune_cfg_p1 - 1) >= 0 || (p.flags & UG_F_GEGLU) || p.R1) return -1;
+  int best = -1; double bfill = 0.0;
+  for (int c = 71; c <= 72; ++c) {
+    const int bm = c == 71 ? 256 : 192;
+    if (!conv_halo_supported(p, batch, bm, 128)) continue;
+    const long tiles = (long)(p.M / bm) * cdiv(p.N, 128);
+    const double fill = (double)tiles / (cdiv(tiles, 256) * 256.0) * (bm == 256 ? 1.0 : 0.97);
+    if (fill > bfill) { bfill = fill; best = c; }
+  }
+  return best;
+}
+
+bool conv_fold_pays(const GemmP& p) {
+  if (p.M < 8192 && !(p.tune_knobs & 67108864)) return false;
+  return true;
+}
+
 void launch_gemm(const GemmP& p0, int batch, hipStream_t s, int* stat_rb) {
   GemmP p = p0;
   if (stat_rb) *stat_rb = 0;
@@ -1294,7 +1312,7 @@
   if (!planned && (p.tune_cfg_p1 - 1) < 0) { int c2, s2; gemm_plan(p0, batch, &c2, &s2); planned = (c2 == cfg && s2 == split); }
   const bool halo_on = planned && !(p.tune_knobs & 16384) && split == 1 && (p.tune_cfg_p1 - 1) < 0 && !(p.flags & UG_F_GEGLU);
   const bool halo_l0 = halo_on && p.N % 160 == 0 && p.N <= 320 && p.C1 == 0 && !(p.tune_knobs & 32768) && conv_halo_supported(p, batch, 256, 128);
-  if (!halo_l0 && planned && p.conv && p.kt == 1 && p.ky == 3 && p.kx == 3 && p.N % 160 == 0 && p.N <= 320 && split == 1 && batch == 1 && !p.up_phase && !(p.flags & (UG_F_OUT_F32 | UG_F_GEGLU)) &&
+  if (!p.S0 && !halo_l0 && planned && p.conv && p.kt == 1 && p.ky == 3 && p.kx == 3 && p.N % 160 == 0 && p.N <= 320 && split == 1 && batch == 1 && !p.up_phase && !(p.flags & (UG_F_OUT_F32 | UG_F_GEGLU)) &&
       (p.tune_cfg_p1 - 1) < 0 && !(p.tune_knobs & 1024) && gemm_can_bufa(p, 64, true)) {
     const long ntn = p.N / 160, tiles = (long)cdiv(p.M, 256) * ntn, whole = tiles / 256 * 256, rem = tiles - whole;
     if (whole > 0 && rem > 0 && rem * 2 <= 256) {
@@ -1333,7 +1351,12 @@
     else if (p.N % 160 == 0 && p.N <= 320) best = -1;
     if (best >= 0) cfg = best;
   }
-  if (planned && !(p.tune_knobs & 65536) && (p.tune_cfg_p1 - 1) < 0 && split == 1 && gemm_stream_supported(p, batch)) {
+  if (p.S0) {
+    const bool forced = (cfg == 71 || cfg == 72) && p0.cfg_p1 - 1 == cfg && conv_halo_supported(p, batch, cfg == 71 ? 256 : 192, 128) && split == 1;
+    if (!forced) cfg = conv_fold_cfg(p, batch, split);
+    UG_REQUIRE(cfg >= 0, "folded shortcut: no halo tile takes this convolution");
+  }
+  if (!p.S0 && planned && !(p.tune_knobs & 65536) && (p.tune_cfg_p1 - 1) < 0 && split == 1 && gemm_stream_supported(p, batch)) {
     cfg = 80;
   }
   if (split > 1) UG_REQUIRE(p.partial != nullptr, "split-K needs a partial buffer");
diff --git a/unigeo_amd/pipeline.py b/unigeo_amd/pipeline.py
--- a/unigeo_amd/pipeline.py
+++ b/unigeo_amd/pipeline.py
@@ -29,7 +29,7 @@
         nbytes = sum(int(np.prod(a.shape)) * 2 for s in (unet_state, vae_state, clip_state) for a in s.values())
         eng = Engine(device_id,
                      workspace_bytes if workspace_bytes is not None else (24 << 30),
-                     persist_bytes if persist_bytes is not None else int(nbytes * 1.35) + (256 << 20))
+                     persist_bytes if persist_bytes is not None else int(nbytes * 1.45) + (256 << 20))
         eng.load_state("unet.", unet_state); eng.bind_unet(u)
         eng.load_state("vae.", vae_state); eng.bind_vae(v)
         eng.load_state("clip.", clip_state); eng.bind_clip(c)
diff --git a/unigeo_amd/stablenormal.py b/unigeo_amd/stablenormal.py
--- a/unigeo_amd/stablenormal.py
+++ b/unigeo_amd/stablenormal.py
@@ -71,7 +71,7 @@
         cfgs = cfgs or (W.SDUNetCfg(), W.VAECfg(), W.DinoCfg())
         nbytes = sum(int(np.prod(a.shape)) * 2 for s in states.values() for a in s.values())
         eng = Engine(device_id, workspace_bytes if workspace_bytes is not None else (24 << 30),
-                     persist_bytes if persist_bytes is not None else int(nbytes * 1.2) + (256 << 20))
+                     persist_bytes if persist_bytes is not None else int(nbytes * 1.3) + (256 << 20))
         for comp in COMPONENTS:
             eng.load_state(f"sn.{comp}.", states[comp])
         eng.bind_stablenormal(*cfgs)
```

New measurement: 28.50 frames/s. Within noise of the previous version (-0.5%).
